# RoadlyInc/DSOPP

Measured on AMD Instinct MI355X. Metric: Gauss-Newton iters/sec (7-KF window, 2k active pts), higher is better.
Workload: dtype f64; 1 GPU; C1: 7-KF window, 2000 active points per GPU (2000 total, 2000 on rank 0), 640x480, full clique, production LM settings; frames=7, points_per_gpu=2000, total_points=2000, parallelism=single GPU, exchange=none, ranks=1

## Files before the change

### dsopp_amd/csrc/pba.hip

```cpp
#include <algorithm>
#include <chrono>
#include <cstdlib>
#include <map>
#include <memory>
#include <mutex>

#include "host_linalg.hpp"
#include "pba_solve_kernels.hpp"
#include "pba_solve_combined.hpp"
#include "pba_schur_two_stage.hpp"
#include "depth_map_kernels.hpp"
#include "point_status_kernels.hpp"
#include "depth_maps.hpp"
#include "activation_kernels.hpp"
#include "immature_set.hpp"
#include "semantic_observation_kernels.hpp"

namespace dsopp_hip {
namespace {

struct ResidualTable {
  DeviceBuffer<uint8_t> status, cand, fej_valid, snap_status;
  DeviceBuffer<double> energy;
  int n = 0, snap_n = 0;
};

struct HostFrame {
  int id = 0;
  int64_t timestamp = 0;
  const dsopp_hip_pyramid *pyramid = nullptr;
  unsigned pyramid_generation = 0;
  int level = 0;
  double intr[4] = {0, 0, 0, 0};
  double exposure = 1;
  bool fixed = false, is_marginalized = false, to_marginalize = false;
  int n = 0;
  int cap = 0;
  std::map<int, std::vector<uint8_t>> pending;
  std::vector<uint8_t> flags;
  DeviceBuffer<double> uv, idepth, idepth_step, idepth_fej, patch, inv_hdd, b_d, relative_baseline, ublk;
  DeviceBuffer<int32_t> n_inliers;
  DeviceBuffer<uint8_t> dflags, snap_flags;
  DeviceBuffer<double> snap_idepth;
  int snap_n = 0;
  std::map<int, std::unique_ptr<ResidualTable>> residuals;
  std::map<int, std::array<double, 36>> covariance;
  std::vector<int> to_internal, to_caller;
  std::vector<int> batch_end;
  DeviceBuffer<int> d_to_internal;
  bool permuted() const { return !to_internal.empty(); }
  DeviceBuffer<uint8_t> sem_hist;
  int internalOf(int caller) const { return to_internal.empty() ? caller : to_internal[static_cast<size_t>(caller)]; }
};

}
}

using namespace dsopp_hip;

struct dsopp_hip_window {
  StreamRef sr;
  dsopp_hip_options opt;
  std::vector<std::unique_ptr<HostFrame>> frames;
  WindowState hst;
  std::vector<double> Hm, bm;
  double energy_marginalized = 0;
  int marg_size = 0;
  DeviceBuffer<FrameDev> d_frames;
  DeviceBuffer<WindowState> d_state, d_state_snap;
  DeviceBuffer<PairConst> d_pc;
  DeviceBuffer<SweepBlock> d_sweep_table;
  DeviceBuffer<SweepBlock> d_fine_table;
  int n_fine_blocks = 0;
  const SweepBlock *fineTable() const { return d_fine_table.ptr ? d_fine_table.ptr : d_sweep_table.ptr; }
  DeviceBuffer<SchurBlock> d_schur_table;
  DeviceBuffer<int> d_pair_first, d_pair_count;
  DeviceBuffer<double> d_partials, d_reduce, d_Hpp, d_bpp, d_Hm, d_Hm_packed, d_bm, d_step, d_scalars, d_gather;
  bool marg_nonzero = false;
  DeviceBuffer<double> d_schur_partials, d_pair_out;
  bool deterministic = false;
  int twoStageMinChunks() const {
    static const int override_chunks = std::getenv("DSOPP_HIP_TWO_STAGE_MIN_CHUNKS") ? std::atoi(std::getenv("DSOPP_HIP_TWO_STAGE_MIN_CHUNKS")) : 0;
    if (override_chunks > 0) return override_chunks;
    return kTwoStageMinChunks;
  }
  bool twoStage() const { return deterministic || n_schur_blocks > twoStageMinChunks(); }
  DeviceMem<unsigned> d_bs_flag;
  unsigned bs_seq = 0, bs_ticket_base = 0;
  PinnedMem<int> h_bs_fault;
  DeviceMem<long long> dbg_stamps;
  DeviceMem<long long> dbg_sweep;
  bool dbg_sweep_lin = true;
  DeviceBuffer<LmControl> d_ctrl;
  const LmControl *fused_final_ctrl = nullptr;
  bool async_pending = false;
  bool begun_with_first_estimate = true;
  int lm_mode = 0;
  double *dHppRaw() const { return d_reduce.ptr; }
  double *dbppRaw() const { return d_reduce.ptr + static_cast<size_t>(K()) * K(); }
  double *dHsc() const { return dbppRaw() + K(); }
  double *dbsc() const { return dHsc() + static_cast<size_t>(K()) * K(); }
  void d_HscDownload(double *host, size_t n, size_t off, hipStream_t st) const {
    HIP_CHECK(hipMemcpyAsync(host, dHsc() + off, n * sizeof(double), hipMemcpyDeviceToHost, st));
  }
  void d_bscDownload(double *host, size_t n, size_t off, hipStream_t st) const {
    HIP_CHECK(hipMemcpyAsync(host, dbsc() + off, n * sizeof(double), hipMemcpyDeviceToHost, st));
  }
  size_t reduceCount() const { return 2 * (static_cast<size_t>(K()) * K() + K()); }
  size_t combCount() const { return static_cast<size_t>(combBlockCount(F())) * 64 + static_cast<size_t>(K()); }
  int comb_copies_active = 1;
  size_t combCopyFirst() const { return (combCount() + 4 * kScalarGroups + 8 + 1) & ~static_cast<size_t>(1); }
  size_t combCopyStride() const { return (combCount() + 1) & ~static_cast<size_t>(1); }
  int n_sweep_blocks = 0, n_schur_blocks = 0;
  bool topology_dirty = true;
  bool frames_dirty = false;
  std::vector<FrameDev> h_frames;
  bool state_dirty = true;
  bool host_stale = false;
  PinnedMem<LmControl> h_ctrl;
  PinnedMem<void> h_uncertainty;
  Event uncertainty_ready;
  bool restore_in_begin = false;
  DeviceBuffer<LmControl> d_results;
  PinnedMem<LmControl> h_results;
  LmControl *result_device = nullptr;
  DeviceBuffer<SelectState> d_select;
  DeviceBuffer<double> d_pair_dist;
  DeviceBuffer<double> d_export;
  PinnedMem<void> h_export;
  struct StageRing {
    PinnedMem<char> mem;
    size_t offset = 0;
  } stage;
  struct AppendOp {
    int kind;
    int n;
    int a;
    int first_block;
    unsigned long long src_off;
    void *dst;
    void *p[6];
  };
  std::vector<uint8_t> append_blob;
  std::vector<AppendOp> append_ops;
  DeviceBuffer<uint8_t> d_append;
  struct ExportEntry {
    int frame_id, n;
    size_t word_offset;
    std::vector<int> target_ids;
  };
  std::vector<ExportEntry> export_entries;
  DeviceBuffer<double> d_update;
  PinnedMem<void> h_update;
  bool export_valid = false;
  std::vector<std::unique_ptr<HostFrame>> frame_pool;
  std::vector<std::unique_ptr<ResidualTable>> table_pool;
  DeviceBuffer<uint8_t> d_sem_args;
  DeviceBuffer<double> dm_tmp;
  std::vector<dsopp_hip_depth_maps *> live_maps;
  struct ActivationScratch {
    DeviceBuffer<ActKeyframe> keyframes;
    DeviceBuffer<ActPair> pairs;
    DeviceBuffer<const void *> texels0;
    DeviceBuffer<double> px, py;
    DeviceBuffer<double> sx, sy;
    DeviceBuffer<int> state, cell_cursor, sid, accepted, nbr, nbr_count;
    DeviceBuffer<double> pack;
  } act;
  bool marg_dirty = true;
  bool pair_valid = false;
  bool begun = false;
  bool linearized = false;
  bool reduced_by_collective = false;
  double last_lambda = 0;
  std::vector<double> last_step;
  float last_solve_ms = 0;
  bool solve_events_pending = false;
  Event ev0, ev1;
  dsopp_hip_allreduce_fn allreduce = nullptr;
  void *allreduce_user = nullptr;
  int rank = 0, world = 1;
  bool profiling = false;
  struct TimedLaunch {
    int cls;
    Event a, b;
  };
  std::vector<TimedLaunch> timed;
  std::vector<Event> event_pool;
  double prof_ms[DSOPP_HIP_NUM_KERNEL_CLASSES] = {0};
  int64_t prof_count[DSOPP_HIP_NUM_KERNEL_CLASSES] = {0};
  WindowState snap_state;
  bool snap_valid = false;
  int snap_F = 0;

  int F() const { return static_cast<int>(frames.size()); }
  int K() const { return kBlk * F(); }
  bool fej() const { return opt.first_estimate_jacobians != 0; }
  int slotOf(int id) const {
    for (size_t i = 0; i < frames.size(); ++i)
      if (frames[i]->id == id) return static_cast<int>(i);
    return -1;
  }
  HostFrame &frameById(int id) {
    const int s = slotOf(id);
    if (s < 0) fail(DSOPP_HIP_ERR_NOT_FOUND, "frame %d is not in the window", id);
    return *frames[static_cast<size_t>(s)];
  }
};

namespace dsopp_hip {
namespace {

using W = dsopp_hip_window;

}
int nativeAllreduce(void *user, void *device_buffer, size_t count, void *stream);
namespace {

Event takeEvent(W &w) {
  Event e;
  if (!w.event_pool.empty()) {
    e = std::move(w.event_pool.back());
    w.event_pool.pop_back();
  } else {
    (void)e.get(hipEventDefault);
  }
  return e;
}

template <typename Body>
void timedLaunch(W &w, int cls, Body &&body) {
  if (!w.profiling) {
    body();
    return;
  }
  Event a = takeEvent(w), b = takeEvent(w);
  HIP_CHECK(hipEventRecord(a.h, w.sr.stream));
  body();
  HIP_CHECK(hipEventRecord(b.h, w.sr.stream));
  w.timed.push_back({cls, std::move(a), std::move(b)});
}

void collectTimings(W &w) {
  if (w.timed.empty()) return;
  w.sr.sync();
  for (auto &t : w.timed) {
    float ms = 0;
    HIP_CHECK(hipEventElapsedTime(&ms, t.a.h, t.b.h));
    w.prof_ms[t.cls] += ms;
    w.prof_count[t.cls] += 1;
    w.event_pool.push_back(std::move(t.a));
    w.event_pool.push_back(std::move(t.b));
  }
  w.timed.clear();
}

__global__ void gatherRowsKernel(const uint8_t *__restrict__ src, uint8_t *__restrict__ dst, const int *__restrict__ rows, int count, int row_bytes) {
  const long long e = static_cast<long long>(blockIdx.x) * blockDim.x + threadIdx.x;
  if (e >= static_cast<long long>(count) * row_bytes) return;
  const int k = static_cast<int>(e / row_bytes), b = static_cast<int>(e % row_bytes);
  dst[e] = src[static_cast<size_t>(rows[k]) * row_bytes + b];
}

void flushAppends(W &w, const char *why = "flush: in front of an entry point");

void splitBatchAt(W &w, HostFrame &f, int n) {
  if (!f.permuted() || n <= 0 || n >= f.n) return;
  int b0 = 0, b1 = f.n;
  for (int e : f.batch_end) {
    if (e == n) return;
    if (e < n) b0 = std::max(b0, e);
    if (e > n) b1 = std::min(b1, e);
  }
  flushAppends(w, "flush: splitBatchAt");
  const int count = b1 - b0;
  std::vector<int> new_to_old;
  new_to_old.reserve(static_cast<size_t>(count));
  for (int p = b0; p < b1; ++p)
    if (f.to_caller[static_cast<size_t>(p)] < n) new_to_old.push_back(p);
  for (int p = b0; p < b1; ++p)
    if (f.to_caller[static_cast<size_t>(p)] >= n) new_to_old.push_back(p);
  hipStream_t st = w.sr.stream;
  DeviceBuffer<int> d_rows;
  DeviceBuffer<uint8_t> tmp;
  d_rows.reserve(static_cast<size_t>(count), 0, st);
  d_rows.upload(new_to_old.data(), new_to_old.size(), 0, st);
  auto permute = [&](void *base, size_t row_bytes) {
    if (!base) return;
    const size_t bytes = static_cast<size_t>(count) * row_bytes;
    tmp.reserve(bytes, 0, st);
    gatherRowsKernel<<<static_cast<unsigned>((bytes + 255) / 256), 256, 0, st>>>(static_cast<const uint8_t *>(base), tmp.ptr, d_rows.ptr, count,
                                                                                 static_cast<int>(row_bytes));
    HIP_CHECK(hipGetLastError());
    HIP_CHECK(hipMemcpyAsync(static_cast<uint8_t *>(base) + static_cast<size_t>(b0) * row_bytes, tmp.ptr, bytes, hipMemcpyDeviceToDevice, st));
  };
  permute(f.uv.ptr, 2 * sizeof(double));
  permute(f.idepth.ptr, sizeof(double));
  permute(f.idepth_step.ptr, sizeof(double));
  permute(f.idepth_fej.ptr, sizeof(double));
  permute(f.patch.ptr, kPat * sizeof(double));
  permute(f.inv_hdd.ptr, sizeof(double));
  permute(f.b_d.ptr, sizeof(double));
  permute(f.relative_baseline.ptr, sizeof(double));
  permute(f.n_inliers.ptr, sizeof(int32_t));
  permute(f.dflags.ptr, 1);
  if (f.ublk.ptr)
    for (int pl = 0; pl < 2 * kMaxFrames; ++pl) permute(f.ublk.ptr + static_cast<size_t>(pl) * ublkPlane(f.cap), kUblk * sizeof(double));
  for (auto &kv : f.residuals) {
    ResidualTable &rt = *kv.second;
    if (rt.n < b1) continue;
    permute(rt.status.ptr, 1);
    permute(rt.cand.ptr, 1);
    permute(rt.fej_valid.ptr, 1);
    permute(rt.energy.ptr, sizeof(double));
  }
  f.snap_n = 0;
  for (auto &kv : f.residuals) kv.second->snap_n = 0;
  w.snap_valid = false;
  HIP_CHECK(hipStreamSynchronize(st));
  const std::vector<int> old_to_caller(f.to_caller.begin() + b0, f.to_caller.begin() + b1);
  for (int k = 0; k < count; ++k) {
    const int c = old_to_caller[static_cast<size_t>(new_to_old[static_cast<size_t>(k)] - b0)];
    f.to_caller[static_cast<size_t>(b0 + k)] = c;
    f.to_internal[static_cast<size_t>(c)] = b0 + k;
  }
  f.batch_end.push_back(n);
  f.d_to_internal.upload(f.to_internal.data(), f.to_internal.size(), 0, st);
  HIP_CHECK(hipStreamSynchronize(st));
  w.linearized = false;
  w.export_valid = false;
}

constexpr int kFirstLandmarkCapacity = 2048;

void ensureLandmarkCapacity(W &w, HostFrame &f, int n) {
  if (n <= f.cap) return;
  flushAppends(w, "flush: landmark arrays grow");
  int cap = f.cap ? f.cap : kFirstLandmarkCapacity;
  while (cap < n) cap *= 2;
  hipStream_t st = w.sr.stream;
  const size_t keep = static_cast<size_t>(f.n);
  f.uv.reserve(2 * static_cast<size_t>(cap), 2 * keep, st);
  f.idepth.reserve(cap, keep, st);
  f.idepth_step.reserve(cap, keep, st);
  f.idepth_fej.reserve(cap, keep, st);
  f.patch.reserve(static_cast<size_t>(kPat) * cap, kPat * keep, st);
  f.inv_hdd.reserve(cap, keep, st);
  f.b_d.reserve(cap, keep, st);
  f.relative_baseline.reserve(cap, keep, st);
  f.n_inliers.reserve(cap, keep, st);
  f.dflags.reserve(cap, keep, st);
  f.ublk.reserve(2 * static_cast<size_t>(kMaxFrames) * ublkPlane(cap), 0, st);
  for (auto &kv : f.residuals) {
    ResidualTable &rt = *kv.second;
    const size_t k = static_cast<size_t>(rt.n);
    rt.status.reserve(cap, k, st);
    rt.cand.reserve(cap, k, st);
    rt.fej_valid.reserve(cap, k, st);
    rt.energy.reserve(cap, k, st);
  }
  f.cap = cap;
  w.topology_dirty = true;
}

void reserveGeometric(PinnedMem<void> &buf, size_t need) {
  if (need <= buf.bytes) return;
  size_t cap = std::max<size_t>(buf.bytes, size_t(1) << 16);
  while (cap < need) cap *= 2;
  buf.reserve(cap);
}

void *stageAcquire(W &w, size_t bytes) {
  bytes = (bytes + 63) & ~static_cast<size_t>(63);
  if (bytes > w.stage.mem.bytes) {
    if (w.stage.mem) {
      w.sr.sync();
      w.stage.mem.reset();
    }
    w.stage.mem.reserve(std::max<size_t>(bytes * 2, size_t(1) << 21));
    w.stage.offset = 0;
  }
  if (w.stage.offset + bytes > w.stage.mem.bytes) {
    w.sr.sync();
    w.stage.offset = 0;
  }
  void *p = w.stage.mem.get() + w.stage.offset;
  w.stage.offset += bytes;
  return p;
}
constexpr int kAppendBlockElems = 2048;

__global__ void __launch_bounds__(256) applyAppendsKernel(const uint8_t *__restrict__ blob, const W::AppendOp *__restrict__ ops, int n_ops) {
  __shared__ int s_op;
  if (threadIdx.x == 0) {
    int lo = 0;
    for (int i = 1; i < n_ops; ++i)
      if (ops[i].first_block <= static_cast<int>(blockIdx.x)) lo = i;
    s_op = lo;
  }
  __syncthreads();
  const W::AppendOp op = ops[s_op];
  const int chunk = static_cast<int>(blockIdx.x) - op.first_block;
  const uint8_t *src = blob + op.src_off;
  const int e0 = chunk * kAppendBlockElems, e1 = e0 + kAppendBlockElems < op.n ? e0 + kAppendBlockElems : op.n;
  if (op.kind == 0) {
    if (op.a == 8) {
      for (int i = e0 + static_cast<int>(threadIdx.x); i < e1; i += 256) static_cast<unsigned long long *>(op.dst)[i] = reinterpret_cast<const unsigned long long *>(src)[i];
    } else if (op.a == 4) {
      for (int i = e0 + static_cast<int>(threadIdx.x); i < e1; i += 256) static_cast<unsigned *>(op.dst)[i] = reinterpret_cast<const unsigned *>(src)[i];
    } else {
      for (int i = e0 + static_cast<int>(threadIdx.x); i < e1; i += 256) static_cast<uint8_t *>(op.dst)[i] = src[i];
    }
    return;
  }
  if (op.kind == 1) {
// ... 2 lines not shown
      const uint8_t h = src[i];
      if (i < op.a) {
        dflags[i] = static_cast<uint8_t>((dflags[i] & (kFlagOutlier | kFlagIllConditioned)) | (h & (kFlagMarginalized | kFlagToMarginalize)));
      } else {
        dflags[i] = h;
        if (op.p[0]) {
          static_cast<double *>(op.p[0])[i] = 0;
          static_cast<double *>(op.p[1])[i] = 0;
          static_cast<double *>(op.p[2])[i] = 0;
          static_cast<double *>(op.p[3])[i] = 0;
          static_cast<double *>(op.p[4])[i] = 0;
          static_cast<int32_t *>(op.p[5])[i] = 0;
        }
      }
    }
    return;
  }
  if (op.kind == 4) {
    const SweepBlock tmpl = *reinterpret_cast<const SweepBlock *>(src);
    const int step = op.a, first = static_cast<int>(reinterpret_cast<intptr_t>(op.p[0])), n_all = static_cast<int>(reinterpret_cast<intptr_t>(op.p[1]));
    SweepBlock *out = static_cast<SweepBlock *>(op.dst);
    for (int k = e0 + static_cast<int>(threadIdx.x); k < e1; k += 256) {
      SweepBlock sb = tmpl;
      sb.offset = k * step * kItemsPerBlock;
      sb.n_groups = n_all ? (step < n_all - k * step ? step : n_all - k * step) : 1;
      sb.partial_row = first + k;
      out[k] = sb;
    }
    return;
  }
  if (op.kind == 3) {
    uint8_t *dflags = static_cast<uint8_t *>(op.dst);
    for (int i = e0 + static_cast<int>(threadIdx.x); i < e1; i += 256) dflags[i] &= static_cast<uint8_t>(~op.a);
    return;
  }
  for (int i = e0 + static_cast<int>(threadIdx.x); i < e1; i += 256) {
    const uint8_t st = src[i];
    const size_t j = static_cast<size_t>(op.a) + static_cast<size_t>(i);
    static_cast<uint8_t *>(op.dst)[j] = st;
    static_cast<uint8_t *>(op.p[0])[j] = st;
    static_cast<uint8_t *>(op.p[1])[j] = 0;
    static_cast<double *>(op.p[2])[j] = 0;
  }
}

void flushAppends(W &w, const char *why) {
  if (w.append_ops.empty()) return;
  HostTimes ht_(why);
  const int n_ops = static_cast<int>(w.append_ops.size());
  int blocks = 0;
  for (W::AppendOp &op : w.append_ops) {
    op.first_block = blocks;
    blocks += (op.n + kAppendBlockElems - 1) / kAppendBlockElems;
  }
  const size_t data_bytes = (w.append_blob.size() + 15) & ~static_cast<size_t>(15), table_bytes = static_cast<size_t>(n_ops) * sizeof(W::AppendOp);
  hipStream_t st = w.sr.stream;
  w.d_append.reserve(data_bytes + table_bytes, 0, st);
  uint8_t *p = static_cast<uint8_t *>(stageAcquire(w, data_bytes + table_bytes));
  std::memcpy(p, w.append_blob.data(), w.append_blob.size());
  std::memcpy(p + data_bytes, w.append_ops.data(), table_bytes);
  HIP_CHECK(hipMemcpyAsync(w.d_append.ptr, p, data_bytes + table_bytes, hipMemcpyHostToDevice, st));
  applyAppendsKernel<<<static_cast<unsigned>(blocks), 256, 0, st>>>(w.d_append.ptr, reinterpret_cast<const W::AppendOp *>(w.d_append.ptr + data_bytes), n_ops);
  HIP_CHECK(hipGetLastError());
  w.append_blob.clear();
  w.append_ops.clear();
}

size_t queueAppendData(W &w, const void *host, size_t bytes, const void *dst_a, const void *dst_b = nullptr) {
  for (const W::AppendOp &op : w.append_ops)
    if (op.dst == dst_a || (dst_b && op.dst == dst_b)) {
      flushAppends(w, "flush: a queued operation writes the same array");
      break;
    }
  const size_t off = (w.append_blob.size() + 7) & ~static_cast<size_t>(7);
  w.append_blob.resize(off + bytes);
  if (bytes) std::memcpy(w.append_blob.data() + off, host, bytes);
  return off;
}

void uploadStagedBytes(W &w, void *dst, const void *host, size_t bytes) {
  if (!bytes) return;
  W::AppendOp op{};
  op.kind = 0;
  const bool words = (bytes & 7) == 0 && (reinterpret_cast<uintptr_t>(dst) & 7) == 0;
  const bool half = (bytes & 3) == 0 && (reinterpret_cast<uintptr_t>(dst) & 3) == 0;
  op.a = words ? 8 : (half ? 4 : 1);
  op.n = static_cast<int>(bytes / static_cast<size_t>(op.a));
  op.src_off = queueAppendData(w, host, bytes, dst);
  op.dst = dst;
  w.append_ops.push_back(op);
}

template <typename T>
void uploadStaged(W &w, DeviceBuffer<T> &dst, const T *host, size_t count, size_t offset) {
  if (!count) return;
  static_assert(sizeof(T) == 8 || sizeof(T) == 4 || sizeof(T) == 1, "element size of a queued copy");
  W::AppendOp op{};
  op.kind = 0;
  op.n = static_cast<int>(count);
  op.a = static_cast<int>(sizeof(T));
  op.src_off = queueAppendData(w, host, count * sizeof(T), dst.ptr + offset);
  op.dst = dst.ptr + offset;
  w.append_ops.push_back(op);
}


void syncTopology(W &w) {
  HostTimes ht_("syncTopology");
  if (!w.topology_dirty) {
    if (w.frames_dirty && w.h_frames.size() == static_cast<size_t>(kMaxFrames) && w.d_frames.ptr) {
      for (int r = 0; r < w.F(); ++r) {
        w.h_frames[static_cast<size_t>(r)].is_marginalized = w.frames[static_cast<size_t>(r)]->is_marginalized;
        w.h_frames[static_cast<size_t>(r)].to_marginalize = w.frames[static_cast<size_t>(r)]->to_marginalize;
      }
      uploadStagedBytes(w, w.d_frames.ptr, w.h_frames.data(), static_cast<size_t>(kMaxFrames) * sizeof(FrameDev));
    }
    w.frames_dirty = false;
    return;
  }
  hipStream_t st = w.sr.stream;
  const int F = w.F();
  static thread_local std::vector<FrameDev> fd;
  static thread_local std::vector<SchurBlock> schur;
  static thread_local std::vector<SweepBlock> pair_tmpl;
  static thread_local std::vector<int> pair_items;
  fd.assign(static_cast<size_t>(kMaxFrames), FrameDev{});
  std::memset(fd.data(), 0, fd.size() * sizeof(FrameDev));
  schur.clear();
  pair_tmpl.resize(kMaxFrames * kMaxFrames);
  pair_items.assign(kMaxFrames * kMaxFrames, 0);
  size_t total_items = 0;
  for (int r = 0; r < F; ++r)
    for (const auto &kv : w.frames[static_cast<size_t>(r)]->residuals) total_items += static_cast<size_t>(kv.second->n);
  const int groups = total_items >= 300000 ? 6 : (total_items >= 30000 ? 4 : 1);
  std::vector<int> pair_first(kMaxFrames * kMaxFrames, -1), pair_count(kMaxFrames * kMaxFrames, 0);
  for (int r = 0; r < F; ++r) {
    HostFrame &f = *w.frames[static_cast<size_t>(r)];
    FrameDev &d = fd[static_cast<size_t>(r)];
    const LevelView lv = f.pyramid->view(f.level);
    d.texels = hbm(lv.texels);
    d.iplane = hbm(f.pyramid->intensityPlane(f.level, st));
    f.pyramid_generation = f.pyramid->generation;
    d.itiles = f.pyramid->itilesX(f.level);
    d.width = lv.width;
    d.height = lv.height;
    d.fx = f.intr[0];
    d.fy = f.intr[1];
    d.cx = f.intr[2];
    d.cy = f.intr[3];
    d.exposure = f.exposure;
    d.fixed = f.fixed;
    d.is_marginalized = f.is_marginalized;
    d.to_marginalize = f.to_marginalize;
    d.n = f.n;
    d.cap = f.cap;
    d.uv = hbm(f.uv.ptr);
    d.idepth = hbm(f.idepth.ptr);
    d.idepth_step = hbm(f.idepth_step.ptr);
    d.idepth_fej = hbm(f.idepth_fej.ptr);
    d.patch = hbm(f.patch.ptr);
    d.inv_hdd = hbm(f.inv_hdd.ptr);
    d.b_d = hbm(f.b_d.ptr);
    d.relative_baseline = hbm(f.relative_baseline.ptr);
    d.n_inliers = hbm(f.n_inliers.ptr);
    d.flags = hbm(f.dflags.ptr);
    d.ublk = hbm(f.ublk.ptr);
    d.snap_idepth = hbm(f.snap_idepth.ptr);
    d.snap_flags = hbm(f.snap_flags.ptr);
    d.first_conn = -1;
    for (int t = 0; t < F; ++t) {
      if (t == r) continue;
      auto it = f.residuals.find(w.frames[static_cast<size_t>(t)]->id);
      if (it == f.residuals.end() || it->second->n == 0) continue;
      ResidualTable &rt = *it->second;
      d.status[t] = hbm(rt.status.ptr);
      d.cand[t] = hbm(rt.cand.ptr);
      d.fej_valid[t] = hbm(rt.fej_valid.ptr);
      d.energy[t] = hbm(rt.energy.ptr);
      d.n_res[t] = rt.n;
      d.snap_status[t] = hbm(rt.snap_status.ptr);
      if (d.first_conn < 0) d.first_conn = t;
      SweepBlock sb;
      std::memset(&sb, 0, sizeof(sb));
      sb.r = r;
      sb.t = t;
      sb.n_res = rt.n;
      sb.cap = f.cap;
      sb.owns_landmark_sums = d.first_conn == t ? 1 : 0;
      sb.width_r = lv.width;
      sb.height_r = lv.height;
      sb.uv = d.uv;
      sb.idepth = d.idepth;
      sb.patch = d.patch;
      sb.idepth_fej = d.idepth_fej;
      sb.b_d = d.b_d;
      sb.inv_hdd = d.inv_hdd;
      sb.idepth_step = d.idepth_step;
      sb.ublk = d.ublk;
      sb.energy = hbm(rt.energy.ptr);
      sb.flags = d.flags;
      sb.status = hbm(rt.status.ptr);
      sb.fej_valid = hbm(rt.fej_valid.ptr);
      sb.cand = hbm(rt.cand.ptr);
      sb.n_groups = 1;
      pair_tmpl[static_cast<size_t>(r * kMaxFrames + t)] = sb;
      pair_items[static_cast<size_t>(r * kMaxFrames + t)] = (rt.n + kItemsPerBlock - 1) / kItemsPerBlock;
    }
    for (int off = 0; off < f.n; off += kSchurLandmarks) {
      SchurBlock sb;
      std::memset(&sb, 0, sizeof(sb));
      sb.r = r;
      sb.offset = off;
      sb.n = d.n;
      sb.cap = d.cap;
      sb.fixed = d.fixed;
      sb.idepth = d.idepth;
      sb.idepth_step = d.idepth_step;
      sb.inv_hdd = d.inv_hdd;
      sb.b_d = d.b_d;
      sb.ublk = d.ublk;
      sb.flags = d.flags;
      for (int t = 0; t < F; ++t) {
        if (d.status[t] == nullptr) continue;
        sb.conn_mask |= 1u << t;
        sb.status[t] = d.status[t];
        sb.cand[t] = d.cand[t];
        sb.n_res[t] = d.n_res[t];
      }
      schur.push_back(sb);
    }
  }
  const int step = groups > 1 ? groups : 1;
  struct PairRange {
    size_t pi;
    int first_sweep, n_sweep, first_fine, n_fine;
  };
  static thread_local std::vector<PairRange> ranges;
  ranges.clear();
  int total_sweep = 0, total_fine = 0;
  for (int t = 0; t < F; ++t)
    for (int r = 0; r < F; ++r) {
      const size_t pi = static_cast<size_t>(r * kMaxFrames + t);
      const int n_all = pair_items[pi];
      if (n_all == 0) continue;
      SweepBlock &tm = pair_tmpl[pi];
      const FrameDev &dr = fd[static_cast<size_t>(r)], &dt = fd[static_cast<size_t>(t)];
      tm.width_t = dt.width;
      tm.height_t = dt.height;
      tm.texels_t = dt.texels;
      tm.iplane_t = dt.iplane;
      tm.itiles_t = dt.itiles;
      for (int k = 0; k < F; ++k)
        if (dr.status[k] != nullptr) tm.conn_mask |= 1u << k;
      const int n_sweep = (n_all + step - 1) / step;
      pair_first[pi] = total_sweep;
      pair_count[pi] = n_sweep;
      ranges.push_back({pi, total_sweep, n_sweep, total_fine, groups > 1 ? n_all : 0});
      total_sweep += n_sweep;
      total_fine += groups > 1 ? n_all : 0;
    }
  w.d_frames.reserve(kMaxFrames, 0, st);
  uploadStagedBytes(w, w.d_frames.ptr, fd.data(), (kMaxFrames) * sizeof(*w.d_frames.ptr));
  w.h_frames = fd;
  w.frames_dirty = false;
  auto queuePairEntries = [&](SweepBlock *table, const SweepBlock &tmpl, int first, int count, int entry_step, int n_all_for_groups) {
    W::AppendOp op{};
    op.kind = 4;
    op.n = count;
    op.a = entry_step;
    op.src_off = queueAppendData(w, &tmpl, sizeof(SweepBlock), table + first);
    op.dst = table + first;
    op.p[0] = reinterpret_cast<void *>(static_cast<intptr_t>(first));
    op.p[1] = reinterpret_cast<void *>(static_cast<intptr_t>(n_all_for_groups));
    w.append_ops.push_back(op);
  };
  const size_t n_sweep_entries = static_cast<size_t>(total_sweep);
  w.n_sweep_blocks = static_cast<int>(n_sweep_entries);
  w.n_schur_blocks = static_cast<int>(schur.size());
  if (n_sweep_entries > w.d_sweep_table.capacity || (groups > 1 && static_cast<size_t>(total_fine) > w.d_fine_table.capacity))
    flushAppends(w, "flush: sweep tables grow");
  w.d_sweep_table.reserve(std::max<size_t>(1, n_sweep_entries), 0, st);
  for (const PairRange &pr : ranges)
    queuePairEntries(w.d_sweep_table.ptr, pair_tmpl[pr.pi], pr.first_sweep, pr.n_sweep, step, groups > 1 ? pair_items[pr.pi] : 0);
  if (groups > 1) {
    w.d_fine_table.reserve(std::max<size_t>(1, static_cast<size_t>(total_fine)), 0, st);
    for (const PairRange &pr : ranges) queuePairEntries(w.d_fine_table.ptr, pair_tmpl[pr.pi], pr.first_fine, pr.n_fine, 1, 0);
    w.n_fine_blocks = total_fine;
  } else {
    w.d_fine_table.release();
    w.n_fine_blocks = static_cast<int>(n_sweep_entries);
  }
  w.d_schur_table.reserve(std::max<size_t>(1, schur.size()), 0, st);
  uploadStagedBytes(w, w.d_schur_table.ptr, schur.data(), (schur.size()) * sizeof(*w.d_schur_table.ptr));
  w.d_pair_first.reserve(kMaxFrames * kMaxFrames, 0, st);
  uploadStagedBytes(w, w.d_pair_first.ptr, pair_first.data(), (pair_first.size()) * sizeof(*w.d_pair_first.ptr));
  w.d_pair_count.reserve(kMaxFrames * kMaxFrames, 0, st);
  uploadStagedBytes(w, w.d_pair_count.ptr, pair_count.data(), (pair_count.size()) * sizeof(*w.d_pair_count.ptr));
  w.d_partials.reserve(std::max<size_t>(1, n_sweep_entries) * kPartial, 0, st);
  w.d_pc.reserve(kMaxFrames * kMaxFrames, 0, st);
  w.d_ctrl.reserve(2, 0, st);
  const size_t KK = static_cast<size_t>(kBlk * kMaxFrames);
  w.d_Hpp.reserve(2 * KK * KK, 0, st);
  w.d_bpp.reserve(KK, 0, st);
  w.d_reduce.reserve(2 * (KK * KK + KK) + 8 + 4 * kScalarGroups + 16 + static_cast<size_t>(kMaxCombCopies - 1) * (static_cast<size_t>(combBlockCount(kMaxFrames)) * 64 + KK + 2), 0, st);
  w.d_Hm.reserve(KK * KK, 0, st);
  w.d_bm.reserve(KK, 0, st);
  w.d_step.reserve(KK, 0, st);
  w.d_scalars.reserve(16 + 4 * kScalarGroups, 0, st);
  w.topology_dirty = false;
  w.pair_valid = false;
}

void uploadState(W &w) {
  if (!w.state_dirty) return;
  w.d_state.reserve(1, 0, w.sr.stream);
  uploadStagedBytes(w, w.d_state.ptr, &w.hst, sizeof(WindowState));
  w.state_dirty = false;
  w.pair_valid = false;
}

void downloadState(W &w) {
  if (w.state_dirty || !w.d_state.ptr || !w.host_stale) return;
  w.host_stale = false;
  w.d_state.download(&w.hst, 1, 0, w.sr.stream);
  w.sr.sync();
}

void uploadMarginal(W &w) {
  if (!w.marg_dirty) return;
  const int K = w.K();
  if (w.marg_size != K) fail(DSOPP_HIP_ERR_STATE, "marginal prior has size %d, window %d", w.marg_size, K);
  w.marg_nonzero = w.energy_marginalized != 0;
  for (double v : w.Hm) w.marg_nonzero = w.marg_nonzero || v != 0;
  for (double v : w.bm) w.marg_nonzero = w.marg_nonzero || v != 0;
  uploadStagedBytes(w, w.d_Hm.ptr, w.Hm.data(), static_cast<size_t>(K) * K * sizeof(double));
  uploadStagedBytes(w, w.d_bm.ptr, w.bm.data(), static_cast<size_t>(K) * sizeof(double));
  const int F = w.F();
  std::vector<double> packed(static_cast<size_t>(combBlockCount(F)) * 64);
  for (int bi = 0; bi < F; ++bi)
    for (int bj = 0; bj <= bi; ++bj)
      for (int i = 0; i < kBlk; ++i)
        for (int j = 0; j < kBlk; ++j)
          packed[static_cast<size_t>(combBlockIndex(bi, bj)) * 64 + static_cast<size_t>(i * kBlk + j)] =
              w.Hm[static_cast<size_t>(kBlk * bi + i) * K + static_cast<size_t>(kBlk * bj + j)];
  w.d_Hm_packed.reserve(static_cast<size_t>(combBlockCount(kMaxFrames)) * 64, 0, w.sr.stream);
  uploadStagedBytes(w, w.d_Hm_packed.ptr, packed.data(), packed.size() * sizeof(double));
  w.marg_dirty = false;
}

void checkPyramidGenerations(W &w) {
  for (const auto &fp : w.frames)
    if (fp->pyramid && fp->pyramid->generation != fp->pyramid_generation) w.topology_dirty = true;
}

void prepare(W &w) {
  w.sr.use();
  checkPyramidGenerations(w);
  downloadState(w);
  syncTopology(w);
  uploadState(w);
  uploadMarginal(w);
  flushAppends(w, "flush: prepare()");
}

void prepareDevice(W &w) {
  w.sr.use();
  flushAppends(w);
  checkPyramidGenerations(w);
  if (w.state_dirty || w.topology_dirty || w.frames_dirty || w.marg_dirty || !w.d_state.ptr) prepare(w);
}

void ensurePairConstants(W &w) {
  if (w.pair_valid) return;
  const int F = w.F();
  timedLaunch(w, DSOPP_HIP_KERNEL_PAIR_SETUP, [&] {
    pairSetupKernel<<<1, kMaxFrames * kMaxFrames, 0, w.sr.stream>>>(w.d_frames.ptr, w.d_state.ptr, w.d_pc.ptr, F, w.fej() ? 1 : 0, nullptr);
  });
  HIP_CHECK(hipGetLastError());
  w.pair_valid = true;
}

template <typename S>
void launchFej(W &w) {
  if (!w.n_sweep_blocks) return;
  timedLaunch(w, DSOPP_HIP_KERNEL_FEJ,
              [&] {
                const int per_wave = 64 / kItemsPerBlock;
                fejKernel<S><<<(w.n_fine_blocks + per_wave - 1) / per_wave, 64, 0, w.sr.stream>>>(w.d_frames.ptr, w.d_pc.ptr, w.fineTable(),
                                                                                                  w.n_fine_blocks);
              });
  HIP_CHECK(hipGetLastError());
}

void firstEstimate(W &w) {
  ensurePairConstants(w);
  if (w.opt.dtype == DSOPP_HIP_F64)
    launchFej<double>(w);
  else
    launchFej<float>(w);
}

struct SweepExtras {
  int ublk_read = 0, ublk_write = 0;
  bool gate_on_pending = false;
  const int *run_flag = nullptr;
  bool fused_lin_backsub = false;
  bool combined = false;
  bool external_backsub = false;
  bool write_fej = false;
};

template <typename S>
void launchSweepTyped(W &w, bool lin, bool huber, bool for_marg, const LmControl *ctrl, bool backsub, double lambda, const SweepExtras &ex) {
  if (!w.n_sweep_blocks) {
    if (lin) HIP_CHECK(hipMemsetAsync(w.d_reduce.ptr, 0, w.reduceCount() * sizeof(double), w.sr.stream));
    return;
  }
  SweepParams prm;
  prm.sigma_huber = w.opt.sigma_huber_loss;
  prm.for_marginalized = for_marg ? 1 : 0;
  prm.use_fej_flag = w.fej() ? 1 : 0;
  prm.ctrl = ctrl;
  prm.clear_buf = lin ? w.d_reduce.ptr : nullptr;
  prm.clear_count = static_cast<int>(ex.combined ? w.combCount() + 4 : w.reduceCount());
  if (ex.combined && w.comb_copies_active > 1)
    prm.clear_count = static_cast<int>(w.combCopyFirst() + (w.comb_copies_active - 1) * w.combCopyStride());
  prm.step = w.d_step.ptr;
  prm.lambda = lambda;
  prm.F = w.F();
  prm.ublk_read = ex.ublk_read;
  prm.ublk_write = ex.ublk_write;
  prm.gate_on_pending = ex.gate_on_pending ? 1 : 0;
  prm.run_flag = ex.run_flag;
  prm.external_backsub = ex.external_backsub ? 1 : 0;
  prm.dbg = (w.dbg_sweep && lin == w.dbg_sweep_lin) ? w.dbg_sweep.get() : nullptr;
  dim3 grid(static_cast<unsigned>(w.n_sweep_blocks)), block(kSweepThreads);
  hipStream_t st = w.sr.stream;
  const FrameDev *fr = w.d_frames.ptr;
  const PairConst *pc = w.d_pc.ptr;
  const SweepBlock *tb = w.d_sweep_table.ptr;
  double *pa = w.d_partials.ptr;
  const bool opening = lin && huber && ex.write_fej && w.fej();
  if (opening) prm.external_backsub = 1;
  timedLaunch(w, lin ? DSOPP_HIP_KERNEL_SWEEP_LINEARIZE : DSOPP_HIP_KERNEL_SWEEP_ENERGY, [&] {
    if (opening) {
      sweepKernel<S, true, true, true, false, true><<<grid, block, 0, st>>>(fr, pc, tb, pa, prm.ctrl, prm.run_flag, prm);
    } else if (lin && ex.fused_lin_backsub) {
      if (w.fej())
        sweepKernel<S, true, true, true, true><<<grid, block, 0, st>>>(fr, pc, tb, pa, prm.ctrl, prm.run_flag, prm);
      else
        sweepKernel<S, true, false, true, true><<<grid, block, 0, st>>>(fr, pc, tb, pa, prm.ctrl, prm.run_flag, prm);
    } else if (!lin && backsub) {
      if (w.fej())
        sweepKernel<S, false, true, true, true><<<grid, block, 0, st>>>(fr, pc, tb, pa, prm.ctrl, prm.run_flag, prm);
      else
        sweepKernel<S, false, false, true, true><<<grid, block, 0, st>>>(fr, pc, tb, pa, prm.ctrl, prm.run_flag, prm);
    } else if (!lin) {
      if (w.fej())
        sweepKernel<S, false, true, true><<<grid, block, 0, st>>>(fr, pc, tb, pa, prm.ctrl, prm.run_flag, prm);
      else
        sweepKernel<S, false, false, true><<<grid, block, 0, st>>>(fr, pc, tb, pa, prm.ctrl, prm.run_flag, prm);
    } else if (w.fej()) {
      if (huber)
        sweepKernel<S, true, true, true><<<grid, block, 0, st>>>(fr, pc, tb, pa, prm.ctrl, prm.run_flag, prm);
      else
        sweepKernel<S, true, true, false><<<grid, block, 0, st>>>(fr, pc, tb, pa, prm.ctrl, prm.run_flag, prm);
    } else {
      if (huber)
        sweepKernel<S, true, false, true><<<grid, block, 0, st>>>(fr, pc, tb, pa, prm.ctrl, prm.run_flag, prm);
      else
        sweepKernel<S, true, false, false><<<grid, block, 0, st>>>(fr, pc, tb, pa, prm.ctrl, prm.run_flag, prm);
    }
  });
  HIP_CHECK(hipGetLastError());
}

void launchSweep(W &w, bool lin, bool huber, bool for_marg, const LmControl *ctrl = nullptr, bool backsub = false, double lambda = 0,
                 const SweepExtras &ex = SweepExtras()) {
  if (!ctrl && !ex.run_flag) ensurePairConstants(w);
  backsub = backsub && w.opt.optimize_idepths;
  if (w.opt.dtype == DSOPP_HIP_F64)
    launchSweepTyped<double>(w, lin, huber, for_marg, ctrl, backsub, lambda, ex);
  else
    launchSweepTyped<float>(w, lin, huber, for_marg, ctrl, backsub, lambda, ex);
}

void allreduceIfNeeded(W &w, double *dev, size_t count) {
  if (!w.allreduce) return;
  const int rc = w.allreduce(w.allreduce_user, dev, count, w.sr.stream);
  if (rc != 0) fail(DSOPP_HIP_ERR_HIP, "allreduce callback failed with %d", rc);
}

size_t schurSmemBytes(int K) {
  const int Kp = (K + 15) & ~15;
  return (static_cast<size_t>(kSchurLandmarks) * schurRowStride(Kp) + 2 * kSchurLandmarks + 40 * static_cast<size_t>(kMaxFrames)) * sizeof(double);
}

struct FusedReduce {
  int ublk_parity;
  LmControl *ctrl_out;
  LmParams prm;
  bool combined = false;
  double comb_lambda = 0;
  const double *scalars = nullptr;
  LmControl *ctrl_host = nullptr;
};

enum class ReduceMode { kFused, kAccumulateOnly, kDecideOnly };
constexpr size_t kDecideSmemBytes = size_t((6 * (kSchurThreads + 2) + 6 * 72) * 8);

void launchTwoStage(W &w, const LmControl *ctrl, int ublk_parity, double lambda, bool dense, double *group_sums);
void launchReduceSchur(W &w, bool for_marg, const LmControl *ctrl, const FusedReduce *fused = nullptr, ReduceMode mode = ReduceMode::kFused) {
  const int K = w.K(), F = w.F();
  hipStream_t st = w.sr.stream;
  if (!fused && !for_marg && !ctrl && w.deterministic) {
    launchTwoStage(w, nullptr, 0, 0.0, true, nullptr);
    allreduceIfNeeded(w, w.d_reduce.ptr, w.reduceCount());
    return;
  }
  ensureDynamicLds(reinterpret_cast<const void *>(reduceSchurKernel), w.sr.device, 96 * 1024);
  ReduceSchurArgs a;
  a.frames = w.d_frames.ptr;
  a.pc = w.d_pc.ptr;
  a.schur_table = w.d_schur_table.ptr;
  a.partials = w.d_partials.ptr;
  a.pair_first_block = w.d_pair_first.ptr;
  a.pair_num_blocks = w.d_pair_count.ptr;
  a.Hpp = w.dHppRaw();
  a.bpp = w.dbppRaw();
  a.Hsc = w.dHsc();
  a.bsc = w.dbsc();
  a.ctrl = ctrl;
  a.F = F;
  a.n_schur_blocks = w.opt.optimize_idepths ? w.n_schur_blocks : 0;
  a.for_marginalized = for_marg ? 1 : 0;
  a.ublk_parity = fused ? fused->ublk_parity : 0;
  a.ctrl_out = (fused && mode != ReduceMode::kAccumulateOnly) ? fused->ctrl_out : nullptr;
  a.st = w.d_state.ptr;
  const bool combined = fused && fused->combined;
  const size_t reduce_count = combined ? w.combCount() : w.reduceCount();
  a.comb = combined ? w.d_reduce.ptr : nullptr;
  a.comb_lambda = fused ? fused->comb_lambda : 0.0;
  if (combined && mode == ReduceMode::kAccumulateOnly && w.comb_copies_active > 1) {
    a.comb_copies = w.comb_copies_active;
    a.comb_copy_first = static_cast<int>(w.combCopyFirst());
    a.comb_copy_stride = static_cast<int>(w.combCopyStride());
  }
  a.scalars = mode == ReduceMode::kDecideOnly ? w.d_reduce.ptr + reduce_count : w.d_scalars.ptr;
  a.n_sweep_blocks = w.n_sweep_blocks;
  a.total_blocks = a.n_schur_blocks + F * F;
  a.scalars_out = mode == ReduceMode::kAccumulateOnly ? w.d_reduce.ptr + reduce_count : nullptr;
  const bool grouped_tail = mode == ReduceMode::kAccumulateOnly && w.allreduce != nullptr;
  a.scalars_out_groups = grouped_tail ? kScalarGroups : 0;
  static_assert(4 * kScalarGroups <= kSchurThreads, "one workgroup writes the grouped tail");
  if (fused) a.prm = fused->prm;
  if (fused && fused->scalars) a.scalars = fused->scalars;
  a.ctrl_host = fused ? fused->ctrl_host : nullptr;
  a.dbg = w.dbg_stamps ? w.dbg_stamps.get() + 24 : nullptr;
  const size_t decide_smem = kDecideSmemBytes;
  if (mode == ReduceMode::kDecideOnly) {
    timedLaunch(w, DSOPP_HIP_KERNEL_ACCEPT,
                [&] { decideApplyKernel<<<std::max(1, a.n_schur_blocks), kSchurThreads, decide_smem, st>>>(a); });
    HIP_CHECK(hipGetLastError());
    return;
  }
  timedLaunch(w, DSOPP_HIP_KERNEL_SCHUR, [&] {
    reduceSchurKernel<<<a.n_schur_blocks + F * F + (a.scalars_out ? 1 : 0), kSchurThreads, std::max(schurSmemBytes(K), decide_smem), st>>>(
        a.ctrl, a.schur_table, a.pc, a.partials, a.pair_first_block, a.pair_num_blocks, a.n_schur_blocks, a.F, a);
  });
  HIP_CHECK(hipGetLastError());
  allreduceIfNeeded(w, w.d_reduce.ptr, reduce_count + (mode == ReduceMode::kAccumulateOnly ? (grouped_tail ? 4 * kScalarGroups : 4) : 0));
  (void)K;
}

SolveArgs makeSolveArgs(W &w) {
  SolveArgs a;
  a.frames = w.d_frames.ptr;
  a.st = w.d_state.ptr;
  a.pc = w.d_pc.ptr;
  a.Hpp_raw = w.dHppRaw();
  a.bpp_raw = w.dbppRaw();
  a.Hpp_out = w.d_Hpp.ptr;
  a.Hsc_copy = w.d_Hpp.ptr + static_cast<size_t>(w.K()) * w.K();
  a.bpp_out = w.d_bpp.ptr;
  a.Hsc = w.dHsc();
  a.bsc = w.dbsc();
  a.use_marginal = w.marg_nonzero ? 1 : 0;
  a.Hm = w.d_Hm.ptr;
  a.bm = w.d_bm.ptr;
  a.step = w.d_step.ptr;
  a.lambda = 0;
  a.affine_reg[0] = w.opt.affine_brightness_regularizer[0];
  a.affine_reg[1] = w.opt.affine_brightness_regularizer[1];
  a.fixed_reg = w.opt.fixed_state_regularizer;
  a.energy_marginalized = w.energy_marginalized;
  a.F = w.F();
  a.fej = w.fej() ? 1 : 0;
  a.do_solve = 1;
  a.store_system = 0;
  a.add_priors = 1;
  return a;
}

size_t solveSmemBytes(int K) {
  const size_t N = static_cast<size_t>(K) + 1;
  return (N * (N + 1) + 4 * static_cast<size_t>(K) + 32 + 38 * static_cast<size_t>(kMaxFrames)) * sizeof(double);
}

void launchAssemble(W &w, double lambda, bool do_solve, bool add_priors, bool store_system) {
  ensureDynamicLds(reinterpret_cast<const void *>(assembleSolveKernel), w.sr.device, 150 * 1024);
  SolveArgs a = makeSolveArgs(w);
  a.lambda = lambda;
  a.do_solve = do_solve ? 1 : 0;
  a.add_priors = add_priors ? 1 : 0;
  a.store_system = store_system ? 1 : 0;
  timedLaunch(w, do_solve ? DSOPP_HIP_KERNEL_ASSEMBLE_SOLVE : DSOPP_HIP_KERNEL_ASSEMBLE,
              [&] { assembleSolveKernel<<<1, kSolveThreads, solveSmemBytes(w.K()), w.sr.stream>>>(a); });
  if (do_solve && !w.fej()) {
    pairSetupKernel<<<1, kMaxFrames * kMaxFrames, 0, w.sr.stream>>>(w.d_frames.ptr, w.d_state.ptr, w.d_pc.ptr, w.F(), 0, nullptr);
  }
  HIP_CHECK(hipGetLastError());
}

void launchTwoStage(W &w, const LmControl *ctrl, int ublk_parity, double lambda, bool dense = false, double *group_sums = nullptr) {
  const int F = w.F();
  hipStream_t st = w.sr.stream;
  using TwoStageKernel = void (*)(TwoStageArgs);
  static const TwoStageKernel kernels[6] = {nullptr, schurTwoStageKernel<2>, schurTwoStageKernel<2>, schurTwoStageKernel<3>, schurTwoStageKernel<4>,
                                            schurTwoStageKernel<5>};
  const int tpw = twoStageTilesPerWave(F);
  if (tpw < 1 || tpw > kMaxTilesPerWave) fail(DSOPP_HIP_ERR_CAPACITY, "window of %d frames exceeds the Schur kernel's tile budget", F);
  const TwoStageKernel two_stage_kernel = kernels[tpw];
  ensureDynamicLds(reinterpret_cast<const void *>(two_stage_kernel), w.sr.device, 96 * 1024);
  const int n_chunks = w.opt.optimize_idepths ? w.n_schur_blocks : 0;
  const int n_wgs = std::max(1, std::min(512, n_chunks));
  w.d_schur_partials.reserve(std::max<size_t>(1, static_cast<size_t>(n_wgs)) * static_cast<size_t>(twoStagePartialCount(F)), 0, st);
  w.d_pair_out.reserve(static_cast<size_t>(kMaxFrames) * kMaxFrames * kPairOut, 0, st);
  TwoStageArgs a;
  a.frames = w.d_frames.ptr;
  a.pc = w.d_pc.ptr;
  a.schur_table = w.d_schur_table.ptr;
  a.partials = w.d_partials.ptr;
  a.dbg = w.dbg_stamps ? w.dbg_stamps.get() + 32 : nullptr;
  a.pair_first_block = w.d_pair_first.ptr;
  a.pair_num_blocks = w.d_pair_count.ptr;
  a.ctrl = ctrl;
  a.schur_partials = w.d_schur_partials.ptr;
  a.pair_out = w.d_pair_out.ptr;
  a.F = F;
  a.n_chunks = n_chunks;
  a.n_schur_wgs = n_wgs;
  a.ublk_parity = ublk_parity;
  a.group_sums = group_sums;
  a.n_sweep_blocks = w.n_sweep_blocks;
  CombineArgs c;
  c.pc = w.d_pc.ptr;
  c.schur_partials = w.d_schur_partials.ptr;
  c.pair_out = w.d_pair_out.ptr;
  c.ctrl = ctrl;
  c.lambda = lambda;
  c.comb = w.d_reduce.ptr;
  c.dense = dense ? w.d_reduce.ptr : nullptr;
  c.F = F;
  c.n_schur_wgs = n_wgs;
  const size_t pair_smem = (48 + 64 + kPairBlk + 8 * 48) * sizeof(double);
  timedLaunch(w, DSOPP_HIP_KERNEL_SCHUR, [&] {
    two_stage_kernel<<<n_wgs + F * F + (group_sums ? kScalarGroups : 0), kSchurThreads, std::max(twoStageSmemBytes(F), pair_smem), st>>>(a);
    combineSystemKernel<<<static_cast<unsigned>((twoStagePartialCount(F) + kCombineEntries - 1) / kCombineEntries), kCombineEntries * kCombineSlices, 0, st>>>(c);
  });
  HIP_CHECK(hipGetLastError());
}

int solveResidentWorkgroups(W &w, bool wide) {
  static std::map<std::pair<int, size_t>, int> cache;
  static std::mutex mu;
  const size_t smem = solveSmemBytes(w.K());
  std::lock_guard<std::mutex> lock(mu);
  const auto key = std::make_pair(w.sr.device * 2 + (wide ? 1 : 0), smem);
  auto it = cache.find(key);
  if (it != cache.end()) return it->second;
  int per_cu = 0, cus = 0;
  if (wide)
    HIP_CHECK(hipOccupancyMaxActiveBlocksPerMultiprocessor(&per_cu, solveCombinedKernel<512>, 512, smem));
  else
    HIP_CHECK(hipOccupancyMaxActiveBlocksPerMultiprocessor(&per_cu, solveCombinedKernel<256>, 256, smem));
  HIP_CHECK(hipDeviceGetAttribute(&cus, hipDeviceAttributeMultiprocessorCount, w.sr.device));
  const int n = std::max(2, per_cu * cus);
  cache[key] = n;
  return n;
}

void launchSolveCombined(W &w, double lambda, LmControl *ctrl, const LmControl *decide_from = nullptr, const LmParams *decide_prm = nullptr,
                         bool decide_from_groups = false, bool backsub = false, int ublk_parity = 0) {
  ensureDynamicLds(reinterpret_cast<const void *>(solveCombinedKernel<256>), w.sr.device, 150 * 1024);
  ensureDynamicLds(reinterpret_cast<const void *>(solveCombinedKernel<256, kMaxCombCopies>), w.sr.device, 150 * 1024);
  ensureDynamicLds(reinterpret_cast<const void *>(solveCombinedKernel<512>), w.sr.device, 150 * 1024);
  SolveCombArgs a;
  if (decide_from) {
    a.dec_in = decide_from;
    a.dec_scalars = w.d_reduce.ptr + w.combCount();
    a.dec_table = w.d_schur_table.ptr;
    a.dec_chunks = w.n_schur_blocks;
    const bool wide = w.F() > 8;
    a.dec_blocks = std::min(wide ? (w.n_schur_blocks + 1) / 2 : w.n_schur_blocks, solveResidentWorkgroups(w, wide) - 1);
    a.dec_groups = decide_from_groups ? kScalarGroups : 0;
    a.dec_prm = *decide_prm;
    if (backsub && a.dec_blocks > 0) {
      if (!w.d_bs_flag) {
        constexpr size_t kHand = static_cast<size_t>(kBlk) * kMaxFrames;
        w.d_bs_flag.alloc(16 + 2 * kHand * sizeof(double));
        std::vector<double> arm(2 * kHand, kHandOverSentinel());
        HIP_CHECK(hipMemsetAsync(w.d_bs_flag.get(), 0, 16, w.sr.stream));
        HIP_CHECK(hipMemcpyAsync(reinterpret_cast<char *>(w.d_bs_flag.get()) + 16, arm.data(), arm.size() * sizeof(double), hipMemcpyHostToDevice, w.sr.stream));
        HIP_CHECK(hipStreamSynchronize(w.sr.stream));
        w.h_bs_fault.reserve(sizeof(int));
        *w.h_bs_fault.get() = 0;
      }
      {
        constexpr size_t kHand = static_cast<size_t>(kBlk) * kMaxFrames;
        double *hand = reinterpret_cast<double *>(reinterpret_cast<char *>(w.d_bs_flag.get()) + 16);
        const unsigned n = w.bs_seq;
        a.bs_ticket = w.d_bs_flag.get();
        a.bs_hand = hand + (n & 1u) * kHand;
        a.bs_hand_next = hand + ((n + 1) & 1u) * kHand;
      }
      a.bs_parity = ublk_parity;
      a.bs_ticket_base = w.bs_ticket_base;
      a.bs_fault = w.h_bs_fault.get();
    }
  }
  a.frames = w.d_frames.ptr;
  a.st = w.d_state.ptr;
  a.pc = w.d_pc.ptr;
  a.comb = w.d_reduce.ptr;
  if (w.comb_copies_active > 1) {
    a.comb_copies = w.comb_copies_active;
    a.comb_copy_first = static_cast<int>(w.combCopyFirst());
    a.comb_copy_stride = static_cast<int>(w.combCopyStride());
  }
  a.Hm = w.d_Hm.ptr;
  a.HmPacked = w.d_Hm_packed.ptr;
  a.bm = w.d_bm.ptr;
  a.step = w.d_step.ptr;
  a.ctrl = ctrl;
  a.lambda = lambda;
  a.affine_reg[0] = w.opt.affine_brightness_regularizer[0];
  a.affine_reg[1] = w.opt.affine_brightness_regularizer[1];
  a.fixed_reg = w.opt.fixed_state_regularizer;
  a.energy_marginalized = w.energy_marginalized;
  a.F = w.F();
  a.fej = w.fej() ? 1 : 0;
  a.use_marginal = w.marg_nonzero ? 1 : 0;
  a.dbg_stamps = w.dbg_stamps.get();
  timedLaunch(w, DSOPP_HIP_KERNEL_ASSEMBLE_SOLVE,
              [&] {
                if (w.F() > 8)
                  solveCombinedKernel<512><<<1 + a.dec_blocks, 512, solveSmemBytes(w.K()), w.sr.stream>>>(
                      a.bs_ticket, a.bs_hand_next, a.dec_in, a.dec_scalars, a.comb, a.frames, a.st, a.F, a);
                else if (a.comb_copies > 1)
                  solveCombinedKernel<256, kMaxCombCopies><<<1 + a.dec_blocks, 256, solveSmemBytes(w.K()), w.sr.stream>>>(
                      a.bs_ticket, a.bs_hand_next, a.dec_in, a.dec_scalars, a.comb, a.frames, a.st, a.F, a);
                else
                  solveCombinedKernel<256><<<1 + a.dec_blocks, 256, solveSmemBytes(w.K()), w.sr.stream>>>(
                      a.bs_ticket, a.bs_hand_next, a.dec_in, a.dec_scalars, a.comb, a.frames, a.st, a.F, a);
              });
  HIP_CHECK(hipGetLastError());
  if (a.bs_ticket) {
    w.bs_seq++;
    w.bs_ticket_base += static_cast<unsigned>(1 + a.dec_blocks);
  }
  if (!w.fej()) {
    pairSetupKernel<<<1, kMaxFrames * kMaxFrames, 0, w.sr.stream>>>(w.d_frames.ptr, w.d_state.ptr, w.d_pc.ptr, w.F(), 0, nullptr);
    HIP_CHECK(hipGetLastError());
  }
}

void checkSolveLaunchFault(W &w) {
  if (!w.h_bs_fault || !*w.h_bs_fault.get()) return;
  *w.h_bs_fault.get() = 0;
  constexpr size_t kHand = static_cast<size_t>(kBlk) * kMaxFrames;
  std::vector<double> arm(2 * kHand, kHandOverSentinel());
  HIP_CHECK(hipMemsetAsync(w.d_bs_flag.get(), 0, 16, w.sr.stream));
  HIP_CHECK(hipMemcpyAsync(reinterpret_cast<char *>(w.d_bs_flag.get()) + 16, arm.data(), arm.size() * sizeof(double), hipMemcpyHostToDevice, w.sr.stream));
  HIP_CHECK(hipStreamSynchronize(w.sr.stream));
  w.bs_seq = 0;
  w.bs_ticket_base = 0;
  fail(DSOPP_HIP_ERR_HIP, "a solve launch's landmark workgroups waited 2 s for the pose step (device shared with a kernel that never yields?): "
                          "the inverse depths of that iteration were not updated, the solve is void");
}

void launchBacksub(W &w, double lambda, const LmControl *ctrl, int ublk_parity = 0, bool gate_on_pending = false) {
  if (!w.opt.optimize_idepths || !w.n_schur_blocks) return;
  timedLaunch(w, DSOPP_HIP_KERNEL_BACKSUB, [&] {
    backsubKernel<<<w.n_schur_blocks, kSchurLandmarks, 0, w.sr.stream>>>(w.d_frames.ptr, w.d_schur_table.ptr, w.d_step.ptr, lambda, w.F(), ctrl,
                                                                         ublk_parity, gate_on_pending ? 1 : 0);
  });
  HIP_CHECK(hipGetLastError());
}


double priorEnergy(const W &w, bool with_step) {
  const int F = w.F(), K = w.K();
  std::vector<double> state(static_cast<size_t>(K));
  for (int f = 0; f < F; ++f)
    for (int a = 0; a < kBlk; ++a) state[static_cast<size_t>(kBlk * f + a)] = w.hst.eps[f][a] + (with_step ? w.hst.step[f][a] : 0.0);
  double e = w.energy_marginalized;
  double quad = 0, lin = 0;
  for (int i = 0; i < K; ++i) {
    lin += w.bm[static_cast<size_t>(i)] * state[static_cast<size_t>(i)];
    double s = 0;
    for (int j = 0; j < K; ++j) s += w.Hm[static_cast<size_t>(i) * K + j] * state[static_cast<size_t>(j)];
    quad += state[static_cast<size_t>(i)] * s;
  }
  e += lin + quad / 2;
  for (int f = 0; f < F; ++f) {
    double t = 0;
    for (int a = 0; a < 2; ++a) {
      const double ab = w.hst.ab0[f][a] + state[static_cast<size_t>(kBlk * f + 6 + a)];
      t += ab * w.opt.affine_brightness_regularizer[a] * ab;
    }
    e += t / 2;
  }
  return e;
}

void stageBegin(W &w) {
  if (w.F() == 0) fail(DSOPP_HIP_ERR_STATE, "window is empty");
  prepare(w);
  if (w.fej()) firstEstimate(w);
  w.begun_with_first_estimate = true;
  w.begun = true;
  w.linearized = false;
}

void fusedBegin(W &w) {
  if (w.F() == 0) fail(DSOPP_HIP_ERR_STATE, "window is empty");
  if (!(w.fej() && w.opt.max_iterations > 0)) {
    stageBegin(w);
    return;
  }
  prepare(w);
  w.begun_with_first_estimate = false;
  w.begun = true;
  w.linearized = false;
}

std::pair<double, int> stageEnergy(W &w) {
  if (!w.begun) fail(DSOPP_HIP_ERR_STATE, "call begin first");
  launchSweep(w, false, true, false);
  timedLaunch(w, DSOPP_HIP_KERNEL_ENERGY_REDUCE,
              [&] { energyReduceKernel<<<1, 256, 0, w.sr.stream>>>(w.d_partials.ptr, w.n_sweep_blocks, w.d_scalars.ptr); });
  HIP_CHECK(hipGetLastError());
  allreduceIfNeeded(w, w.d_scalars.ptr, 2);
  double out[2];
  w.d_scalars.download(out, 2, 0, w.sr.stream);
  w.sr.sync();
  return {out[0] + priorEnergy(w, true), static_cast<int>(out[1] + 0.5)};
}

void stageLinearize(W &w, bool huber = true, bool for_marg = false, bool add_priors = true) {
  if (!w.begun) fail(DSOPP_HIP_ERR_STATE, "call begin first");
  launchSweep(w, true, huber, for_marg);
  launchReduceSchur(w, for_marg, nullptr);
  launchAssemble(w, 0.0, false, add_priors, true);
  w.linearized = true;
}

void stageStep(W &w, double lambda) {
  if (!w.linearized) fail(DSOPP_HIP_ERR_STATE, "call linearize first");
  launchAssemble(w, lambda, true, true, false);
  w.pair_valid = true;
  launchBacksub(w, lambda, nullptr);
  const int K = w.K();
  w.last_step.resize(static_cast<size_t>(K));
  w.d_step.download(w.last_step.data(), static_cast<size_t>(K), 0, w.sr.stream);
  w.sr.sync();
  for (int f = 0; f < w.F(); ++f)
    for (int a = 0; a < kBlk; ++a) w.hst.step[f][a] = -w.last_step[static_cast<size_t>(kBlk * f + a)];
  w.last_lambda = lambda;
}

std::pair<double, double> stageAccept(W &w, bool accept) {
  HIP_CHECK(hipMemsetAsync(w.d_scalars.ptr + 4, 0, 4 * sizeof(double), w.sr.stream));
  timedLaunch(w, DSOPP_HIP_KERNEL_ACCEPT, [&] {
    if (w.n_schur_blocks) {
      acceptLandmarksKernel<<<w.n_schur_blocks, kSchurThreads, 0, w.sr.stream>>>(w.d_frames.ptr, w.d_schur_table.ptr, w.F(), accept ? 1 : 0,
                                                                                  w.d_scalars.ptr + 4);
    }
    acceptFramesKernel<<<1, 128, 0, w.sr.stream>>>(w.d_state.ptr, w.F(), accept ? 1 : 0, w.d_scalars.ptr + 6);
  });
  HIP_CHECK(hipGetLastError());
  if (accept) allreduceIfNeeded(w, w.d_scalars.ptr + 4, 2);
  double n4[4];
  w.d_scalars.download(n4, 4, 4, w.sr.stream);
  w.sr.sync();
  const double norms[2] = {n4[0] + n4[2], n4[1] + n4[3]};
  for (int f = 0; f < w.F(); ++f)
    for (int a = 0; a < kBlk; ++a) {
      if (accept) w.hst.eps[f][a] += w.hst.step[f][a];
      w.hst.step[f][a] = 0;
    }
  if (!accept) w.pair_valid = false;
  return {norms[0], norms[1]};
}

void restoreHostSide(W &w) {
  if (!w.snap_valid || w.snap_F != w.F()) fail(DSOPP_HIP_ERR_STATE, "no snapshot matching the current window");
  w.sr.use();
  flushAppends(w);
  for (auto &fp : w.frames) {
    if (fp->snap_n != fp->n) fail(DSOPP_HIP_ERR_STATE, "frame %d changed since the snapshot", fp->id);
    for (auto &kv : fp->residuals)
      if (kv.second->snap_n != kv.second->n) fail(DSOPP_HIP_ERR_STATE, "connection of frame %d changed since the snapshot", fp->id);
  }
  syncTopology(w);
  flushAppends(w);
  w.hst = w.snap_state;
  w.state_dirty = false;
  w.host_stale = false;
  w.pair_valid = false;
  w.begun = false;
}

void launchRestore(W &w) {
  restoreKernel<<<w.n_schur_blocks + 1, kSchurLandmarks, 0, w.sr.stream>>>(w.d_frames.ptr, w.d_schur_table.ptr, w.F(), w.d_state.ptr, w.d_state_snap.ptr,
                                                                        w.n_schur_blocks);
  HIP_CHECK(hipGetLastError());
}

void lmSolveFusedEnqueue(W &w) {
  hipStream_t st = w.sr.stream;
  LmParams prm;
  prm.function_tolerance = w.opt.function_tolerance;
  prm.parameter_tolerance = w.opt.parameter_tolerance;
  prm.decrease_on_accept = 1.0;
  prm.increase_on_reject = 1.0;
  prm.lambda0 = 1.0 / w.opt.initial_trust_region_radius;
  prm.max_iterations = w.opt.max_iterations;
  prm.min_iterations = 3;
  prm.force_accept = w.opt.force_accept;
  prm.use_reduced_scalars = w.allreduce ? 1 : 0;
  LmControl *ctrl = w.d_ctrl.ptr;
  const bool sweep_takes_fej = w.fej() && w.opt.max_iterations > 0 && !w.begun_with_first_estimate;
  const bool begin_sets_pairs = !w.pair_valid;
  {
    LmInitArgs ia;
    ia.pair_frames = begin_sets_pairs ? w.d_frames.ptr : nullptr;
    ia.pair_pc = w.d_pc.ptr;
    ia.pair_fej = w.fej() ? 1 : 0;
    w.pair_valid = true;
    ia.sa = makeSolveArgs(w);
    ia.schur_table = w.d_schur_table.ptr;
    ia.n_schur_blocks = w.n_schur_blocks;
    ia.ctrl = ctrl;
    ia.prm = prm;
    int begin_blocks = 1;
    if (w.restore_in_begin) {
      w.restore_in_begin = false;
      if (begin_sets_pairs) {
        ia.restore_state = w.d_state.ptr;
        ia.sa.st = w.d_state_snap.ptr;
        begin_blocks += w.n_schur_blocks + 1;
      } else {
        launchRestore(w);
      }
    }
    lmBeginKernel<<<begin_blocks, kSolveThreads, (static_cast<size_t>(w.K()) + 16) * sizeof(double), st>>>(ia);
  }
  HIP_CHECK(hipGetLastError());
  const int rounds = (w.opt.force_accept ? w.opt.max_iterations : 2 * w.opt.max_iterations) + 1;
  bool result_written_by_kernel = false;
  const bool k3_backsub = w.opt.optimize_idepths && w.n_schur_blocks > 0;
  static const int comb_copies_min_chunks = std::getenv("DSOPP_HIP_COMB_COPIES_MIN_CHUNKS") ? std::atoi(std::getenv("DSOPP_HIP_COMB_COPIES_MIN_CHUNKS")) : 80;
  w.comb_copies_active = (!w.twoStage() && !w.allreduce && w.F() <= 7 && w.n_schur_blocks >= comb_copies_min_chunks) ? kMaxCombCopies : 1;
  struct CopiesReset {
    W &w;
    ~CopiesReset() { w.comb_copies_active = 1; }
  } copies_reset{w};
  for (int r = 0; r < rounds; ++r) {
    LmControl *cin = ctrl + (r & 1), *cout = ctrl + ((r + 1) & 1);
    SweepExtras ex;
    ex.ublk_read = (r + 1) & 1;
    ex.ublk_write = r & 1;
    ex.gate_on_pending = true;
    ex.fused_lin_backsub = true;
    ex.combined = true;
    ex.write_fej = r == 0 && sweep_takes_fej;
    const bool large = w.n_schur_blocks > w.twoStageMinChunks();
    if (k3_backsub) {
      ex.fused_lin_backsub = false;
      ex.external_backsub = true;
      launchSweep(w, r + 1 < rounds, true, false, cin, false, 0.0, ex);
    } else if (large && r + 1 == rounds) {
      launchBacksub(w, 0.0, cin, ex.ublk_read, true);
      ex.fused_lin_backsub = false;
      ex.external_backsub = true;
      launchSweep(w, false, true, false, cin, false, 0.0, ex);
    } else if (large) {
      if (r > 0) launchBacksub(w, 0.0, cin, ex.ublk_read, true);
      ex.fused_lin_backsub = false;
      ex.external_backsub = true;
      launchSweep(w, true, true, false, cin, false, 0.0, ex);
    } else {
      launchSweep(w, r + 1 < rounds, true, false, cin, true, 0.0, ex);
    }
    FusedReduce fr;
    fr.ublk_parity = r & 1;
    fr.ctrl_out = cout;
    fr.prm = prm;
    fr.combined = true;
    bool decide_from_groups = false;
    if (w.twoStage() && r + 1 < rounds) {
      double *groups = w.d_reduce.ptr + w.combCount();
      launchTwoStage(w, cin, fr.ublk_parity, 0.0, false, groups);
      allreduceIfNeeded(w, w.d_reduce.ptr, w.combCount() + 4 * kScalarGroups);
      decide_from_groups = true;
    } else if (w.allreduce && r + 1 == rounds) {
      if (large) {
        sweepScalarGroupsKernel<<<kScalarGroups, 256, 0, st>>>(w.d_partials.ptr, w.n_sweep_blocks, w.d_scalars.ptr + 16, cin);
        sweepScalarGroupsFinalKernel<<<1, 64, 0, st>>>(w.d_scalars.ptr + 16, w.d_reduce.ptr + w.combCount());
      } else {
        sweepScalarsKernel<<<1, 256, 0, st>>>(w.d_partials.ptr, w.n_sweep_blocks, w.d_reduce.ptr + w.combCount(), cin);
      }
      HIP_CHECK(hipGetLastError());
      allreduceIfNeeded(w, w.d_reduce.ptr + w.combCount(), 4);
      launchReduceSchur(w, false, cin, &fr, ReduceMode::kDecideOnly);
    } else if (r + 1 == rounds) {
      w.h_ctrl.reserve(sizeof(LmControl));
      fr.ctrl_host = w.result_device ? w.result_device : w.h_ctrl.get();
      result_written_by_kernel = true;
      if (large) {
        sweepScalarGroupsKernel<<<kScalarGroups, 256, 0, st>>>(w.d_partials.ptr, w.n_sweep_blocks, w.d_scalars.ptr + 16, cin);
        HIP_CHECK(hipGetLastError());
        fr.prm.use_reduced_scalars = 2;
        fr.scalars = w.d_scalars.ptr + 16;
      }
      launchReduceSchur(w, false, cin, &fr, ReduceMode::kDecideOnly);
    } else {
      launchReduceSchur(w, false, cin, &fr, ReduceMode::kAccumulateOnly);
      decide_from_groups = w.allreduce != nullptr;
    }
    if (r + 1 < rounds) launchSolveCombined(w, 0.0, cout, cin, &fr.prm, decide_from_groups, k3_backsub, fr.ublk_parity);
  }
  LmControl *cfin = ctrl + (rounds & 1);
  HIP_CHECK(hipGetLastError());
  w.pair_valid = false;
  w.h_ctrl.reserve(sizeof(LmControl));
  if (!result_written_by_kernel) {
    if (w.result_device)
      HIP_CHECK(hipMemcpyAsync(w.result_device, cfin, sizeof(LmControl), hipMemcpyDeviceToDevice, st));
    else
      HIP_CHECK(hipMemcpyAsync(w.h_ctrl.get(), cfin, sizeof(LmControl), hipMemcpyDeviceToHost, st));
  }
  w.host_stale = true;
  w.fused_final_ctrl = cfin;
}

void lmSolveFusedFinish(W &w, double &energy_out, int &iterations, int &n_valid_out) {
  hipStream_t st = w.sr.stream;
  const LmControl *cfin = w.fused_final_ctrl;
  w.sr.sync();
  checkSolveLaunchFault(w);
  if (w.h_ctrl.get()->need_final_setup) {
    ensurePairConstants(w);
    launchSweep(w, false, true, false);
    HIP_CHECK(hipGetLastError());
    w.sr.sync();
  }
  (void)st;
  (void)cfin;
  energy_out = w.h_ctrl.get()->energy;
  iterations = w.h_ctrl.get()->iteration;
  n_valid_out = w.h_ctrl.get()->n_valid;
}

void lmSolveFused(W &w, double &energy_out, int &iterations, int &n_valid_out) {
  lmSolveFusedEnqueue(w);
  lmSolveFusedFinish(w, energy_out, iterations, n_valid_out);
}

}
}

namespace dsopp_hip {
namespace {

Rigid poseOf(const W &w, int f) {
  Rigid T0;
  for (int i = 0; i < 9; ++i) T0.R[i] = w.hst.T0_R[f][i];
  for (int i = 0; i < 3; ++i) T0.t[i] = w.hst.T0_t[f][i];
  return rigidMul(T0, rigidExp(w.hst.eps[f]));
}

void relinearize(W &w) {
  prepareDevice(w);
  relinearizeKernel<<<1, kMaxFrames * kMaxFrames, 0, w.sr.stream>>>(w.d_frames.ptr, w.d_state.ptr, w.d_pc.ptr, w.F(), w.fej() ? 1 : 0, w.F() - 1);
  HIP_CHECK(hipGetLastError());
  w.host_stale = true;
  w.pair_valid = true;
}

void updatePointStatusesDevice(W &w) {
  prepareDevice(w);
  hipStream_t st = w.sr.stream;
  const int F = w.F();
  if (!w.d_select.ptr) {
    w.d_select.reserve(1, 0, st);
    selectInitKernel<<<1, 1024, 0, st>>>(w.d_select.ptr);
  }
  w.d_pair_dist.reserve(static_cast<size_t>(kMaxFrames) * kMaxFrames, 0, st);
  const double half_sigma_sq = w.opt.sigma_huber_loss * w.opt.sigma_huber_loss / 2;
  if (w.n_sweep_blocks) {
    const int per_group = kSelectThreads / kItemsPerBlock;
    const int grid = (w.n_fine_blocks + per_group - 1) / per_group;
    for (int pass = kSelectPasses - 1; pass >= 0; --pass)
      selectHistKernel<<<grid, kSelectThreads, 0, st>>>(w.d_frames.ptr, w.fineTable(), w.n_fine_blocks, w.d_select.ptr, pass);
  }
  pairDistanceKernel<<<1, 256, 0, st>>>(w.d_state.ptr, F, w.d_pair_dist.ptr, w.n_sweep_blocks ? w.d_select.ptr : nullptr, half_sigma_sq);
  if (w.n_schur_blocks)
    applyPointStatusesKernel<<<w.n_schur_blocks, kSchurLandmarks, 0, st>>>(w.d_frames.ptr, w.d_schur_table.ptr, F, w.d_select.ptr, w.d_pair_dist.ptr);
  HIP_CHECK(hipGetLastError());
}

void updatePointStatuses(W &w) {
  if (!(w.allreduce && w.world > 1)) {
    updatePointStatusesDevice(w);
    return;
  }
  prepare(w);
  downloadState(w);
  const int F = w.F();
  hipStream_t st = w.sr.stream;
  struct Conn {
    int r, t;
    std::vector<uint8_t> status, cand;
    std::vector<double> energy;
  };
  std::vector<Conn> conns;
  std::vector<std::vector<uint8_t>> flags(static_cast<size_t>(F));
  std::vector<std::vector<double>> idepth(static_cast<size_t>(F)), baseline(static_cast<size_t>(F));
  for (int r = 0; r < F; ++r) {
    HostFrame &f = *w.frames[static_cast<size_t>(r)];
    flags[static_cast<size_t>(r)].resize(static_cast<size_t>(f.n));
    idepth[static_cast<size_t>(r)].resize(static_cast<size_t>(f.n));
    baseline[static_cast<size_t>(r)].resize(static_cast<size_t>(f.n));
    f.dflags.download(flags[static_cast<size_t>(r)].data(), static_cast<size_t>(f.n), 0, st);
    f.idepth.download(idepth[static_cast<size_t>(r)].data(), static_cast<size_t>(f.n), 0, st);
    f.relative_baseline.download(baseline[static_cast<size_t>(r)].data(), static_cast<size_t>(f.n), 0, st);
    for (int t = 0; t < F; ++t) {
      if (t == r) continue;
      HostFrame &g = *w.frames[static_cast<size_t>(t)];
      if (g.is_marginalized) continue;
      auto it = f.residuals.find(g.id);
      if (it == f.residuals.end() || it->second->n == 0) continue;
      Conn c;
      c.r = r;
      c.t = t;
      c.status.resize(static_cast<size_t>(it->second->n));
      c.cand.resize(static_cast<size_t>(it->second->n));
      c.energy.resize(static_cast<size_t>(it->second->n));
      it->second->status.download(c.status.data(), c.status.size(), 0, st);
      it->second->cand.download(c.cand.data(), c.cand.size(), 0, st);
      it->second->energy.download(c.energy.data(), c.energy.size(), 0, st);
      conns.push_back(std::move(c));
    }
  }
  w.sr.sync();
  std::vector<double> energies;
  for (const Conn &c : conns)
    for (size_t i = 0; i < c.status.size(); ++i) {
      if (flags[static_cast<size_t>(c.r)][i] & kFlagMarginalized) continue;
      if (c.status[i] == DSOPP_HIP_STATUS_OK) energies.push_back(c.energy[i]);
    }
  if (w.allreduce && w.world > 1) {
    std::vector<double> counts(static_cast<size_t>(w.world), 0.0);
    counts[static_cast<size_t>(w.rank)] = static_cast<double>(energies.size());
    w.d_gather.reserve(static_cast<size_t>(w.world), 0, st);
    w.d_gather.upload(counts.data(), counts.size(), 0, st);
    allreduceIfNeeded(w, w.d_gather.ptr, counts.size());
    w.d_gather.download(counts.data(), counts.size(), 0, st);
    w.sr.sync();
    size_t total = 0, offset = 0;
    for (int r = 0; r < w.world; ++r) {
      if (r < w.rank) offset += static_cast<size_t>(counts[static_cast<size_t>(r)] + 0.5);
      total += static_cast<size_t>(counts[static_cast<size_t>(r)] + 0.5);
    }
    std::vector<double> all(total, 0.0);
    std::copy(energies.begin(), energies.end(), all.begin() + static_cast<long>(offset));
    if (total) {
      w.d_gather.reserve(total, 0, st);
      w.d_gather.upload(all.data(), total, 0, st);
      allreduceIfNeeded(w, w.d_gather.ptr, total);
      w.d_gather.download(all.data(), total, 0, st);
      w.sr.sync();
    }
    energies.swap(all);
  }
  double threshold = 0;
  if (!energies.empty()) {
    const size_t q = static_cast<size_t>(static_cast<double>(energies.size()) * 0.75);
    std::nth_element(energies.begin(), energies.begin() + static_cast<long>(q), energies.end());
    threshold = energies[q] + w.opt.sigma_huber_loss * w.opt.sigma_huber_loss / 2;
  }
  std::vector<std::vector<int32_t>> inliers(static_cast<size_t>(F));
  std::vector<std::vector<int>> valid(static_cast<size_t>(F));
  for (int r = 0; r < F; ++r) {
    inliers[static_cast<size_t>(r)].assign(static_cast<size_t>(w.frames[static_cast<size_t>(r)]->n), 0);
    valid[static_cast<size_t>(r)].assign(static_cast<size_t>(w.frames[static_cast<size_t>(r)]->n), 0);
  }
  for (Conn &c : conns) {
    const Rigid Tr = poseOf(w, c.r), Tt = poseOf(w, c.t);
    const double dx = Tr.t[0] - Tt.t[0], dy = Tr.t[1] - Tt.t[1], dz = Tr.t[2] - Tt.t[2];
    const double distance = std::sqrt(dx * dx + dy * dy + dz * dz);
    for (size_t i = 0; i < c.status.size(); ++i) {
      if (flags[static_cast<size_t>(c.r)][i] & kFlagMarginalized) continue;
      if (c.energy[i] > threshold) {
        c.status[i] = DSOPP_HIP_STATUS_OUTLIER;
        c.cand[i] = DSOPP_HIP_STATUS_OUTLIER;
        c.energy[i] = 0;
      }
      if (c.status[i] == DSOPP_HIP_STATUS_OK) {
        double &bl = baseline[static_cast<size_t>(c.r)][i];
        bl = std::max(bl, idepth[static_cast<size_t>(c.r)][i] * distance);
        valid[static_cast<size_t>(c.r)][i]++;
        inliers[static_cast<size_t>(c.r)][i]++;
      }
    }
    ResidualTable &rt = *w.frames[static_cast<size_t>(c.r)]->residuals[w.frames[static_cast<size_t>(c.t)]->id];
    rt.status.upload(c.status.data(), c.status.size(), 0, st);
    rt.cand.upload(c.cand.data(), c.cand.size(), 0, st);
    rt.energy.upload(c.energy.data(), c.energy.size(), 0, st);
  }
  for (int r = 0; r < F; ++r) {
    HostFrame &f = *w.frames[static_cast<size_t>(r)];
    bool any_conn = false;
    for (const Conn &c : conns) any_conn = any_conn || c.r == r;
    for (int i = 0; i < f.n; ++i) {
      uint8_t &fl = flags[static_cast<size_t>(r)][static_cast<size_t>(i)];
      if (fl & kFlagMarginalized) continue;
      if (valid[static_cast<size_t>(r)][static_cast<size_t>(i)] < 1) fl |= kFlagOutlier;
    }
    (void)any_conn;
    f.dflags.upload(flags[static_cast<size_t>(r)].data(), static_cast<size_t>(f.n), 0, st);
    f.relative_baseline.upload(baseline[static_cast<size_t>(r)].data(), static_cast<size_t>(f.n), 0, st);
    std::vector<int32_t> cur(static_cast<size_t>(f.n));
    f.n_inliers.download(cur.data(), cur.size(), 0, st);
    w.sr.sync();
    for (int i = 0; i < f.n; ++i)
      if (!(flags[static_cast<size_t>(r)][static_cast<size_t>(i)] & kFlagMarginalized)) cur[static_cast<size_t>(i)] = inliers[static_cast<size_t>(r)][static_cast<size_t>(i)];
    f.n_inliers.upload(cur.data(), cur.size(), 0, st);
    w.sr.sync();
    f.flags.resize(static_cast<size_t>(f.n));
    for (int c = 0; c < f.n; ++c) f.flags[static_cast<size_t>(c)] = flags[static_cast<size_t>(r)][static_cast<size_t>(f.internalOf(c))];
  }
  w.sr.sync();
}

bool estimateUncertaintyEnqueue(W &w, bool force_state) {
  prepareDevice(w);
  if (w.fej()) firstEstimate(w);
  w.begun = true;
  stageLinearize(w, false, false, true);
  const int K = w.K();
  const size_t kk = static_cast<size_t>(K) * K;
  const bool want_state = force_state || (w.host_stale && !w.state_dirty);
  const size_t bytes = 2 * kk * sizeof(double) + sizeof(WindowState);
  reserveGeometric(w.h_uncertainty, bytes);
  const hipEvent_t ready = w.uncertainty_ready.get(hipEventDisableTiming);
  double *Hpp = static_cast<double *>(w.h_uncertainty.get()), *Hsc = Hpp + kk;
  w.d_Hpp.download(Hpp, 2 * kk, 0, w.sr.stream);
  if (want_state) HIP_CHECK(hipMemcpyAsync(Hsc + kk, w.d_state.ptr, sizeof(WindowState), hipMemcpyDeviceToHost, w.sr.stream));
  HIP_CHECK(hipEventRecord(ready, w.sr.stream));
  return want_state;
}

void estimateUncertaintyHost(W &w, bool want_state);

void estimateUncertainty(W &w) {
  const bool want_state = estimateUncertaintyEnqueue(w, false);
  estimateUncertaintyHost(w, want_state);
}
// ... 2029 lines not shown
```

### dsopp_amd/csrc/pba_solve_combined.hpp

```cpp
#pragma once
#include "pba_solve_kernels.hpp"

namespace dsopp_hip {

struct SolveCombArgs {
  const FrameDev *frames;
  WindowState *st;
  PairConst *pc;
  const double *comb;
  int comb_copies = 1;
  int comb_copy_first = 0, comb_copy_stride = 0;
  const double *Hm, *bm;
  const double *HmPacked = nullptr;
  double *step;
  LmControl *ctrl;
  double lambda;
  double affine_reg[2];
  double fixed_reg;
  double energy_marginalized;
  int F;
  int fej;
  int use_marginal;
  long long *dbg_stamps;
  const LmControl *dec_in = nullptr;
  const double *dec_scalars = nullptr;
  const SchurBlock *dec_table = nullptr;
  int dec_blocks = 0;
  int dec_groups = 0;
  LmParams dec_prm;
  unsigned *bs_ticket = nullptr;
  double *bs_hand = nullptr;
  double *bs_hand_next = nullptr;
  int bs_parity = 0;
  int dec_chunks = 0;
  unsigned bs_ticket_base = 0;
  int *bs_fault = nullptr;
};
__host__ __device__ inline double kHandOverSentinel() {
  union {
    unsigned long long u;
    double d;
  } c;
  c.u = 0x7FF8D50FF00DBEEFull;
  return c.d;
}
constexpr int kMaxCombCopies = 4;
#define SC_STAMP(i) do { if (kStamps && a.dbg_stamps && tid == 0) a.dbg_stamps[i] = wall_clock64(); } while (0)

__device__ __forceinline__ void combBlockDecode(int b, int &bi, int &bj) {
  int r = static_cast<int>((__fsqrt_rn(8.0f * static_cast<float>(b) + 1.0f) - 1.0f) * 0.5f);
  if ((r + 1) * (r + 2) / 2 <= b) ++r;
  if (r * (r + 1) / 2 > b) --r;
  bi = r;
  bj = b - r * (r + 1) / 2;
}

template <int THREADS, int COPIES = 1>
__global__ void __launch_bounds__(THREADS, 1) solveCombinedKernel(unsigned *bs_ticket_p, double *bs_hand_next_p, const LmControl *dec_in_p,
                                                                  const double *dec_scalars_p, const double *comb_p, const FrameDev *frames_p,
                                                                  WindowState *st_p, int F_p, SolveCombArgs a) {
  extern __shared__ __attribute__((aligned(16))) char smem_raw[];
  const int F = F_p, K = kBlk * F;
  const int N = K + 1;
  const int ld = N + 1;
  double *A = reinterpret_cast<double *>(smem_raw);
  double *pv = A + N * ld;
  double *xs = pv + K;
  double *Linv = xs + K + 16;
  double *epsl = Linv + 36 * kMaxFrames;
  double *stpl = epsl + K;
  double *ab0l = stpl + K;
  const int tid = threadIdx.x;
  const int wave = tid >> 6, lane = tid & 63;
  const long long sc_t_entry = (kStamps && a.dbg_stamps) ? wall_clock64() : 0;

  int c_active = 1, c_relin = 0;
  double lam = a.lambda;
  const bool decides = dec_in_p != nullptr;
  double dec_eps = 0, dec_step = 0;
  int dec_accept = 0;
  const bool ticketed = bs_ticket_p != nullptr;
  unsigned ticket_raw = 0;
  if (ticketed && tid == 0) {
    auto tp = glb(bs_ticket_p);
    asm volatile("" : "+v"(tp));
    ticket_raw = __hip_atomic_fetch_add(tp, 1u, __ATOMIC_RELAXED, __HIP_MEMORY_SCOPE_AGENT);
  }
  if (ticketed && tid < kBlk * kMaxFrames) bs_hand_next_p[tid] = kHandOverSentinel();
  const void DSOPP_CONSTANT *any_words = (const void DSOPP_CONSTANT *)__builtin_amdgcn_kernarg_segment_ptr();
  const LmControl DSOPP_CONSTANT *cin_src = dec_in_p ? (const LmControl DSOPP_CONSTANT *)dec_in_p : (const LmControl DSOPP_CONSTANT *)any_words;
  static_assert(sizeof(a) >= sizeof(LmControl) && sizeof(a) >= 4 * sizeof(double), "the argument block stands in for an absent control block / scalar block");
  static_assert(sizeof(LmControl) == 6 * sizeof(double) + 8 * sizeof(int), "LmControl changed: extend the scalar copy below");
  LmControl cin;
  cin.lambda = cin_src->lambda;
  cin.energy = cin_src->energy;
  cin.cand_prior = cin_src->cand_prior;
  cin.idepth_sq = cin_src->idepth_sq;
  cin.frame_state_sq = cin_src->frame_state_sq;
  cin.frame_step_sq = cin_src->frame_step_sq;
  cin.n_valid = cin_src->n_valid;
  cin.converged = cin_src->converged;
  cin.active = cin_src->active;
  cin.linear_system_valid = cin_src->linear_system_valid;
  cin.iteration = cin_src->iteration;
  cin.need_final_setup = cin_src->need_final_setup;
  cin.pending = cin_src->pending;
  cin.relin = cin_src->relin;
  const double DSOPP_CONSTANT *t_src = dec_scalars_p ? (const double DSOPP_CONSTANT *)dec_scalars_p : (const double DSOPP_CONSTANT *)any_words;
  double t_early[4] = {t_src[0], t_src[1], t_src[2], t_src[3]};
  asm volatile("" : "+s"(cin.lambda), "+s"(cin.energy), "+s"(cin.cand_prior), "+s"(cin.idepth_sq), "+s"(cin.frame_state_sq), "+s"(cin.frame_step_sq),
               "+s"(cin.n_valid), "+s"(cin.converged), "+s"(cin.active), "+s"(cin.linear_system_valid), "+s"(cin.iteration),
               "+s"(cin.need_final_setup), "+s"(cin.pending), "+s"(cin.relin), "+s"(t_early[0]), "+s"(t_early[1]), "+s"(t_early[2]), "+s"(t_early[3])
               : "s"(a.pc), "s"(a.Hm), "s"(a.bm), "s"(a.HmPacked), "s"(a.step), "s"(a.ctrl), "s"(a.fej), "s"(a.use_marginal), "s"(a.dec_table),
               "s"(a.dec_blocks), "s"(a.dec_groups), "s"(a.bs_hand), "s"(a.bs_parity), "s"(a.dec_chunks), "s"(a.bs_ticket_base), "s"(a.comb_copies),
               "s"(a.comb_copy_first), "s"(a.comb_copy_stride), "s"(a.lambda), "s"(a.affine_reg[0]), "s"(a.affine_reg[1]), "s"(a.fixed_reg),
               "s"(a.energy_marginalized));
  __shared__ unsigned s_vblock;
  bool main_wg = ticketed || blockIdx.x == 0;
  struct {
    int valid;
    Rigid T0;
    double fxr, fyr, cxr, cyr, fxt, fyt, cxt, cyt, exposure_r, exposure_t;
  } pp;
  pp.valid = 0;
  const bool fast_refresh = a.fej != 0;
  auto requestPairInputs = [&] {
    if (fast_refresh && tid < F * F) {
      const int r = tid / F, t = tid - F * (tid / F);
      const PairConst &P = a.pc[r * kMaxFrames + t];
      pp.valid = P.valid;
#pragma unroll
      for (int i = 0; i < 3; ++i) {
#pragma unroll
        for (int j = 0; j < 3; ++j) pp.T0.R[3 * i + j] = P.T0rel[4 * i + j];
        pp.T0.t[i] = P.T0rel[4 * i + 3];
      }
      const FrameDev &fr = frames_p[r];
      const FrameDev &ft = frames_p[t];
      pp.fxr = fr.fx;
      pp.fyr = fr.fy;
      pp.cxr = fr.cx;
      pp.cyr = fr.cy;
      pp.fxt = ft.fx;
      pp.fyt = ft.fy;
      pp.cxt = ft.cx;
      pp.cyt = ft.cy;
      pp.exposure_r = fr.exposure;
      pp.exposure_t = ft.exposure;
    }
  };
  double eps_c = 0, ab0_c = 0, rhs_c = 0, bm_c = 0;
  int fixed_c = 0, tomarg_c = 0;
  if (main_wg && tid < K) {
    const int f = tid >> 3, i = tid & 7;
    if (!decides) eps_c = st_p->eps[f][i];
    if (decides) {
      dec_eps = st_p->eps[f][i];
      dec_step = st_p->step[f][i];
    }
    fixed_c = frames_p[f].fixed;
    tomarg_c = frames_p[f].to_marginalize;
    ab0_c = st_p->ab0[f][i < 6 ? 0 : i - 6];
    rhs_c = comb_p[combBlockCount(F) * 64 + tid];
    if (COPIES > 1) {
      for (int cp = 1; cp < a.comb_copies; ++cp)
        rhs_c += comb_p[a.comb_copy_first + static_cast<size_t>(cp - 1) * a.comb_copy_stride + combBlockCount(F) * 64 + tid];
    }
    if (a.use_marginal) bm_c = a.bm[tid];
  }
  const int pc = tid - 64;
  const bool prior_thread = main_wg && pc >= 0 && pc < K;
  double ab0_p = 0, bm_p = 0;
  auto requestTailInputs = [&] {
    if (prior_thread) {
      ab0_p = st_p->ab0[pc >> 3][(pc & 7) < 6 ? 0 : (pc & 7) - 6];
      if (a.use_marginal) bm_p = a.bm[pc];
    }
  };
  if (!ticketed) requestTailInputs();
  const int n_entries = combBlockCount(F) * 64;
  constexpr int kBatch = THREADS >= 512 ? 6 : 8;
  double hv[kBatch], hm[kBatch];
  auto loadBatch = [&](int base) {
#pragma unroll
    for (int u = 0; u < kBatch; ++u) {
      const int e = base + tid + THREADS * u;
      hv[u] = comb_p[min(e, n_entries - 1)];
      hm[u] = 0;
    }
    if (COPIES > 1) {
      double hc[COPIES > 1 ? COPIES - 1 : 1][kBatch];
#pragma unroll
      for (int cp = 1; cp < COPIES; ++cp) {
        const double *cpy = comb_p + a.comb_copy_first + static_cast<size_t>(cp - 1) * a.comb_copy_stride;
#pragma unroll
        for (int u = 0; u < kBatch; ++u) hc[cp - 1][u] = 0;
        if (cp < a.comb_copies) {
#pragma unroll
          for (int u = 0; u < kBatch; ++u) hc[cp - 1][u] = cpy[min(base + tid + THREADS * u, n_entries - 1)];
        }
      }
#pragma unroll
      for (int cp = 1; cp < COPIES; ++cp)
#pragma unroll
        for (int u = 0; u < kBatch; ++u) hv[u] += hc[cp - 1][u];
    }
    if (a.use_marginal) {
#pragma unroll
      for (int u = 0; u < kBatch; ++u) hm[u] = a.HmPacked[min(base + tid + THREADS * u, n_entries - 1)];
    }
  };
  if (main_wg) loadBatch(0);
  if (decides) {
    __shared__ LmControl s_dec_out;
    __shared__ int s_dec_accept, s_dec_proceed;
    double t[4] = {0, 0, 0, 0};
    if (a.dec_groups) {
      __shared__ double s_grp[4 * 8];
      if (tid < 32) {
        const int e = tid >> 3, j = tid & 7;
        const auto gsrc = glb(dec_scalars_p);
        double gv[8];
#pragma unroll
        for (int k = 0; k < 8; ++k) gv[k] = gsrc[4 * (8 * j + k) + e];
        asm volatile("" : "+v"(gv[0]), "+v"(gv[1]), "+v"(gv[2]), "+v"(gv[3]), "+v"(gv[4]), "+v"(gv[5]), "+v"(gv[6]), "+v"(gv[7]));
        double sacc = 0;
#pragma unroll
        for (int k = 0; k < 8; ++k) sacc += gv[k];
        s_grp[e * 8 + j] = sacc;
      }
      ldsBarrier();
      if (tid == 0) {
#pragma unroll
        for (int e = 0; e < 4; ++e) {
          double sacc = 0;
#pragma unroll
          for (int j = 0; j < 8; ++j) sacc += s_grp[e * 8 + j];
          t[e] = sacc;
        }
      }
    } else {
      t[0] = t_early[0];
      t[1] = t_early[1];
      t[2] = t_early[2];
      t[3] = t_early[3];
    }
    if (!cin.active) {
      if (tid == 0 && (ticketed ? ticket_raw == a.bs_ticket_base : blockIdx.x == 0)) *a.ctrl = cin;
      return;
    }
    SC_STAMP(8);
    if (tid == 0) {
      LmControl c;
      int accept = 0, proceed = 0;
      lmDecision(cin, t, a.dec_prm, c, accept, proceed);
      s_dec_out = c;
      s_dec_accept = accept;
      s_dec_proceed = proceed;
      s_vblock = ticketed ? ticket_raw - a.bs_ticket_base : blockIdx.x;
    }
    ldsBarrier();
    SC_STAMP(9);
    dec_accept = s_dec_accept;
    const unsigned vblock = s_vblock;
    main_wg = vblock == 0;
    if (vblock > 0) {
      constexpr int LP = THREADS / 4, CPP = LP / kSchurLandmarks;
      static_assert(CPP >= 1, "a pass covers whole chunks");
      const int W = gridDim.x - 1, n_pass = (a.dec_chunks + CPP - 1) / CPP;
      const int sub = tid & 3, grp = tid >> 2, l = grp & (kSchurLandmarks - 1), chunk_in_pass = grp / kSchurLandmarks;
      if (cin.pending) {
        for (int p = static_cast<int>(vblock) - 1; p < n_pass; p += W) {
          const int chunk = p * CPP + chunk_in_pass;
          if (chunk >= a.dec_chunks) continue;
          const SchurBlock &be = a.dec_table[chunk];
          const int i = be.offset + l;
          if (i >= be.n) continue;
#pragma unroll
          for (int h = 0; h < 4; ++h) {
            const int t2 = sub + 4 * h;
            if (t2 < F && be.status[t2] != nullptr && i < be.n_res[t2]) {
              if (dec_accept)
                be.status[t2][i] = be.cand[t2][i];
              else
                be.cand[t2][i] = be.status[t2][i];
            }
          }
          if (sub == 0) {
            if (dec_accept) be.idepth[i] += be.idepth_step[i];
            be.idepth_step[i] = 0;
          }
        }
      }
      if (!ticketed || !s_dec_proceed || s_dec_out.relin) return;
      auto backSubstitute = [&](auto ns_tag) {
      constexpr int NS = decltype(ns_tag)::value;
      constexpr int kPre = THREADS >= 512 ? (NS >= 4 ? 1 : 2) : 2;
      double rows[kPre][NS][kBlk], bdv[kPre], ihv[kPre];
      hbm_f64 *dstp[kPre];
    #pragma unroll
      for (int u = 0; u < kPre; ++u) {
        dstp[u] = nullptr;
        bdv[u] = ihv[u] = 0;
    #pragma unroll
        for (int q = 0; q < NS; ++q)
    #pragma unroll
          for (int c = 0; c < kBlk; ++c) rows[u][q][c] = 0;
      }
      auto fetch = [&](int p, double (&rw)[NS][kBlk], double &bd, double &ih, hbm_f64 *&dst) {
        dst = nullptr;
        const int chunk = p * CPP + chunk_in_pass;
        if (chunk >= a.dec_chunks) return;
        const SchurBlock &be = a.dec_table[chunk];
        const int i = be.offset + l;
        if (i >= be.n) return;
        const uint8_t flg = be.flags[i];
        if (flg & (kFlagMarginalized | kFlagIllConditioned)) return;
        const size_t plane = ublkPlane(be.cap);
        const hbm_f64 *base = be.ublk + static_cast<size_t>(a.bs_parity) * kMaxFrames * plane + static_cast<size_t>(i) * kUblk;
    #pragma unroll
        for (int q = 0; q < NS; ++q) {
          int t = sub + 4 * q;
          asm volatile("" : "+v"(t));
          if (t < F && (t == be.r || ((be.conn_mask >> t) & 1u))) {
    #pragma unroll
            for (int c = 0; c < kBlk; ++c) rw[q][c] = base[t * plane + c];
          }
        }
        bd = be.b_d[i];
        ih = be.inv_hdd[i];
        dst = be.idepth_step + i;
      };
    #pragma unroll
      for (int u = 0; u < kPre; ++u) {
        const int p = static_cast<int>(vblock) - 1 + u * W;
        if (p < n_pass) fetch(p, rows[u], bdv[u], ihv[u], dstp[u]);
      }
      double *stp = reinterpret_cast<double *>(smem_raw);
      __shared__ int s_timed_out;
      if (tid == 0) s_timed_out = 0;
      ldsBarrier();
      if (tid < kBlk * kMaxFrames) {
        double v = 0;
        if (tid < K) {
          const long long t0 = wall_clock64();
          for (;;) {
            v = __hip_atomic_load(a.bs_hand + tid, __ATOMIC_RELAXED, __HIP_MEMORY_SCOPE_AGENT);
            if (__double_as_longlong(v) != __double_as_longlong(kHandOverSentinel())) break;
            __builtin_amdgcn_s_sleep(24);
            if (wall_clock64() - t0 > 200000000ll) {
              s_timed_out = 1;
              if (a.bs_fault) __hip_atomic_store(a.bs_fault, 1, __ATOMIC_RELAXED, __HIP_MEMORY_SCOPE_SYSTEM);
              break;
            }
          }
        }
        stp[tid] = v;
      }
      __syncthreads();
      if (s_timed_out) return;
      const double damp = 1.0 / (1.0 + s_dec_out.lambda);
      auto finish = [&](const double (&rw)[NS][kBlk], double bd, double ih, hbm_f64 *dst) {
        double d = 0;
    #pragma unroll
        for (int q = 0; q < NS; ++q) {
          const double *sq = stp + kBlk * (sub + 4 * q);
    #pragma unroll
          for (int c = 0; c < kBlk; ++c) d += rw[q][c] * sq[c];
        }
        d += dppMove<0xB1>(d);
        d += dppMove<0x4E>(d);
        if (sub == 0 && dst) *dst = -((bd - d) * damp * ih);
      };
    #pragma unroll
      for (int u = 0; u < kPre; ++u) finish(rows[u], bdv[u], ihv[u], dstp[u]);
      for (int p = static_cast<int>(vblock) - 1 + kPre * W; p < n_pass; p += W) {
        double rw[NS][kBlk], bd = 0, ih = 0;
        hbm_f64 *dst = nullptr;
    #pragma unroll
        for (int q = 0; q < NS; ++q)
    #pragma unroll
          for (int c = 0; c < kBlk; ++c) rw[q][c] = 0;
        fetch(p, rw, bd, ih, dst);
        finish(rw, bd, ih, dst);
      }
      };
      if (THREADS < 512)
        backSubstitute(std::integral_constant<int, 2>{});
      else if (F <= 12)
        backSubstitute(std::integral_constant<int, 3>{});
      else
        backSubstitute(std::integral_constant<int, 4>{});
      return;
    }
    if (cin.pending && tid < K) {
      if (dec_accept) {
        dec_eps += dec_step;
        st_p->eps[tid >> 3][tid & 7] = dec_eps;
      }
      st_p->step[tid >> 3][tid & 7] = 0;
    }
    if (tid == 64) *a.ctrl = s_dec_out;
    if (!s_dec_proceed) return;
    c_active = 1;
    c_relin = s_dec_out.relin;
    lam = s_dec_out.lambda;
  } else if (a.ctrl) {
    c_active = a.ctrl->active;
    c_relin = a.ctrl->relin;
    lam = a.ctrl->lambda;
  }
  if (decides) eps_c = dec_eps;
  SC_STAMP(0);
  if (kStamps && a.dbg_stamps && tid == 0) a.dbg_stamps[7] = sc_t_entry;
  asm volatile("" : "+v"(fixed_c), "+v"(tomarg_c), "+v"(c_active), "+v"(c_relin));
  int prior_kind = 0;
  double pd_c = 0;
  if (tid < K) {
    if (!tomarg_c) prior_kind = fixed_c ? 1 : ((tid & 7) >= 6 ? 2 : 0);
    pd_c = prior_kind == 1 ? a.fixed_reg : (prior_kind == 2 ? ((tid & 7) == 6 ? a.affine_reg[0] : a.affine_reg[1]) : 0.0);
    xs[tid] = eps_c;
    epsl[tid] = eps_c;
    Linv[tid] = pd_c;
    if ((tid & 7) >= 6) ab0l[2 * (tid >> 3) + (tid & 7) - 6] = ab0_c;
  }
  ldsBarrier();
  SC_STAMP(10);
  if (!c_active || c_relin) return;
  const double *prior_diag = Linv;
  const int in_row = (tid >> 3) & 7, in_col = tid & 7;
  double *const A_thr = A + in_row * ld + in_col;
  auto storeBatch = [&](int base) {
    int blk = __builtin_amdgcn_readfirstlane((base + tid) >> 6);
    int bi, bj;
    combBlockDecode(blk, bi, bj);
    bi = __builtin_amdgcn_readfirstlane(bi);
    bj = __builtin_amdgcn_readfirstlane(bj);
    const int n_blocks = n_entries >> 6;
#pragma unroll
    for (int u = 0; u < kBatch; ++u) {
      if (blk < n_blocks) {
        const int blk_off = __builtin_amdgcn_readfirstlane(8 * bi * ld + 8 * bj);
        const double v = hv[u] + hm[u];
        if (bi != bj) {
          A_thr[blk_off] = v;
        } else if (in_col <= in_row) {
          double vd = v;
          if (in_row == in_col) {
            const int row = 8 * bi + in_row;
            vd += prior_diag[row] * (1.0 + lam);
            pv[row] = vd + 10.0;
          }
          A_thr[blk_off] = vd;
        }
      }
      blk += THREADS / 64;
      bj += THREADS / 64;
      while (bj > bi) {
        bj -= bi + 1;
        ++bi;
      }
    }
  };
  storeBatch(0);
  for (int base = kBatch * THREADS; base < n_entries; base += kBatch * THREADS) {
    loadBatch(base);
    storeBatch(base);
  }
  SC_STAMP(11);
  if (tid < K) {
    double v = rhs_c;
    if (prior_kind == 1)
      v += a.fixed_reg * eps_c;
    else if (prior_kind == 2)
      v += ((tid & 7) == 6 ? a.affine_reg[0] : a.affine_reg[1]) * (ab0_c + eps_c);
    if (a.use_marginal) {
      double s = 0;
      for (int k = 0; k < K; ++k) s += a.Hm[tid * K + k] * xs[k];
      v += bm_c + s;
    }
    A[K * ld + tid] = v;
  }
  if (tid == 0) A[K * ld + K] = 0;
  ldsBarrier();
  SC_STAMP(1);
  if (main_wg) requestPairInputs();

  choleskyAugmented<THREADS>(A, pv, Linv, F, tid, a.dbg_stamps);
  SC_STAMP(2);
  if (ticketed) requestTailInputs();
  if (wave == 0) {
    backSubstituteWave(A, Linv, xs, F, lane);
    SC_STAMP(6);
  }
  __syncthreads();
  if (tid < K) {
    const double x = xs[tid];
    stpl[tid] = -x;
    if (a.bs_hand) __hip_atomic_store(a.bs_hand + tid, x, __ATOMIC_RELAXED, __HIP_MEMORY_SCOPE_AGENT);
    a.step[tid] = x;
    st_p->step[tid >> 3][tid & 7] = -x;
  }
  SC_STAMP(3);
  double part = 0, nstate = 0, nstep = 0;
  auto priorMath = [&] {
    if (!a.ctrl || !prior_thread) return;
    const double xc = epsl[pc] + stpl[pc];
    if (a.use_marginal) {
      double sacc = 0;
      for (int k = 0; k < K; ++k) sacc += a.Hm[pc * K + k] * (epsl[k] + stpl[k]);
      part += bm_p * xc + 0.5 * xc * sacc;
    }
    if ((pc & 7) >= 6) {
      const double ab = ab0_p + xc;
      part += 0.5 * ab * ((pc & 7) == 6 ? a.affine_reg[0] : a.affine_reg[1]) * ab;
    }
    nstate = epsl[pc] * epsl[pc] + ((pc & 7) >= 6 ? ab0_p * ab0_p : 0.0);
    nstep = stpl[pc] * stpl[pc];
  };
  if (fast_refresh) {
    ldsBarrier();
    Rigid *E = reinterpret_cast<Rigid *>(A);
    if (tid < 2 * F) {
      const int f = tid < F ? tid : tid - F;
      const double sign = tid < F ? 1.0 : -1.0;
      double xi[6];
#pragma unroll
      for (int i = 0; i < 6; ++i) xi[i] = sign * (epsl[kBlk * f + i] + stpl[kBlk * f + i]);
      E[tid] = rigidExp(xi);
    }
    ldsBarrier();
    asm volatile("" : "+v"(pp.valid));
    if (tid < F * F && pp.valid) {
      const int r = tid / F, t = tid - F * (tid / F);
      PairConst &P = a.pc[r * kMaxFrames + t];
      const Rigid T_tr = rigidMul(E[F + t], rigidMul(pp.T0, E[r]));
      const double ifx = 1.0 / pp.fxr, ify = 1.0 / pp.fyr;
      const double k02 = -pp.cxr * ifx, k12 = -pp.cyr * ify;
      double U[12];
#pragma unroll
      for (int i = 0; i < 3; ++i) {
        U[4 * i + 0] = T_tr.R[3 * i + 0] * ifx;
        U[4 * i + 1] = T_tr.R[3 * i + 1] * ify;
        U[4 * i + 2] = T_tr.R[3 * i + 0] * k02 + T_tr.R[3 * i + 1] * k12 + T_tr.R[3 * i + 2];
        U[4 * i + 3] = T_tr.t[i];
      }
#pragma unroll
      for (int j = 0; j < 4; ++j) {
        P.M[0 + j] = pp.fxt * U[0 + j] + pp.cxt * U[8 + j];
        P.M[4 + j] = pp.fyt * U[4 + j] + pp.cyt * U[8 + j];
        P.M[8 + j] = U[8 + j];
      }
      const double a_r = ab0l[2 * r] + epsl[kBlk * r + 6] + stpl[kBlk * r + 6];
      const double a_t = ab0l[2 * t] + epsl[kBlk * t + 6] + stpl[kBlk * t + 6];
      P.s = (pp.exposure_t / pp.exposure_r) * exp(a_t - a_r);
      P.b_t = ab0l[2 * t + 1] + epsl[kBlk * t + 7] + stpl[kBlk * t + 7];
      P.b_r = ab0l[2 * r + 1] + epsl[kBlk * r + 7] + stpl[kBlk * r + 7];
    }
    priorMath();
  } else {
    ldsBarrier();
    priorMath();
  }
  SC_STAMP(4);
  if (a.ctrl && K <= 64) {
    if (wave == 1) {
      part = waveSum(part);
      nstate = waveSum(nstate);
      nstep = waveSum(nstep);
      if (tid == 64) {
        a.ctrl->cand_prior = a.energy_marginalized + part;
        a.ctrl->frame_state_sq = nstate;
        a.ctrl->frame_step_sq = nstep;
        a.ctrl->pending = 1;
      }
    }
  } else if (a.ctrl) {
    part = waveSum(part);
    nstate = waveSum(nstate);
    nstep = waveSum(nstep);
    ldsBarrier();
    if ((tid & 63) == 0) {
      xs[tid >> 6] = part;
      xs[THREADS / 64 + (tid >> 6)] = nstate;
      xs[2 * (THREADS / 64) + (tid >> 6)] = nstep;
    }
    ldsBarrier();
    if (tid == 64) {
      constexpr int kWaves = THREADS / 64;
      double total = a.energy_marginalized, s_state = 0, s_step = 0;
      for (int w = 0; w < kWaves; ++w) {
        total += xs[w];
        s_state += xs[kWaves + w];
        s_step += xs[2 * kWaves + w];
      }
      a.ctrl->cand_prior = total;
      a.ctrl->frame_state_sq = s_state;
      a.ctrl->frame_step_sq = s_step;
      a.ctrl->pending = 1;
    }
  }
  SC_STAMP(5);
}

}
```

### dsopp_amd/csrc/pba_solve_kernels.hpp

```cpp
#pragma once
#include <cstddef>
#include <type_traits>
#include "pba_kernels.hpp"

namespace dsopp_hip {


struct LmParams {
  double function_tolerance, parameter_tolerance;
  double decrease_on_accept, increase_on_reject;
  double lambda0;
  int max_iterations, min_iterations;
  int force_accept;
  int use_reduced_scalars;
};

constexpr int kSchurLandmarks = 64;
constexpr int kSchurThreads = 512;
constexpr int kPairBlk = 144;

__host__ __device__ inline int schurRowStride(int Kp) {
  return ((Kp + 15) / 32) * 32 + 16;
}

__device__ inline void derivePairBlocks(const double *__restrict__ G , const PairConst &P, double *__restrict__ out ,
                                        double *lds , int lane) {
  const int i = lane >> 3, j = lane & 7;
  double gt;
  if (j < 6) {
    gt = 0;
#pragma unroll
    for (int k = 0; k < 6; ++k) gt += G[symIdx(i, k)] * P.Adj[6 * k + j];
  } else if (j == 6) {
    gt = G[symIdx(i, 6)];
  } else {
    gt = G[symIdx(i, 7)] * P.s0;
  }
  lds[lane] = gt;
  out[64 + lane] = gt;
  __builtin_amdgcn_s_waitcnt(0);
  __builtin_amdgcn_wave_barrier();
  double tgt;
  if (i < 6) {
    tgt = 0;
#pragma unroll
    for (int k = 0; k < 6; ++k) tgt += P.Adj[6 * k + i] * lds[8 * k + j];
  } else if (i == 6) {
    tgt = lds[48 + j];
  } else {
    tgt = P.s0 * lds[56 + j];
  }
  out[lane] = tgt;
  if (lane < 8) {
    const double *q = G + 36;
    double s;
    if (lane < 6) {
      s = 0;
#pragma unroll
      for (int k = 0; k < 6; ++k) s += P.Adj[6 * k + lane] * q[k];
    } else if (lane == 6) {
      s = q[6];
    } else {
      s = P.s0 * q[7];
    }
    out[128 + lane] = s;
  }
}

__host__ __device__ constexpr int combBlockIndex(int bi, int bj) { return bi * (bi + 1) / 2 + bj; }
__host__ __device__ constexpr int combBlockCount(int F) { return F * (F + 1) / 2; }
__device__ __forceinline__ int combIndex(int row, int col) { return combBlockIndex(row >> 3, col >> 3) * 64 + ((row & 7) << 3) + (col & 7); }

struct ReduceSchurArgs {
  const FrameDev *frames;
  const PairConst *pc;
  const SchurBlock *schur_table;
  const double *partials;
  const int *pair_first_block, *pair_num_blocks;
  double *Hpp, *bpp;
  double *Hsc, *bsc;
  const LmControl *ctrl;
  int F;
  int n_schur_blocks;
  int for_marginalized;
  int ublk_parity;
  LmControl *ctrl_out;
  WindowState *st;
  const double *scalars;
  int n_sweep_blocks;
  int total_blocks;
  double *scalars_out;
  int scalars_out_groups = 0;
  double *comb;
  int comb_copies = 1;
  int comb_copy_first = 0, comb_copy_stride = 0;
  double comb_lambda;
  LmParams prm;
  long long *dbg;
  LmControl *ctrl_host = nullptr;
};
#define RS_STAMP(i) do { if (kStamps && a.dbg && threadIdx.x == 0 && blockIdx.x == 1) a.dbg[i] = wall_clock64(); } while (0)

using f64x4 = __attribute__((ext_vector_type(4))) double;

constexpr int kScalarGroups = 64;

struct ApplyRegs {
  uint8_t *p_status[2], *p_cand[2];
  uint8_t v_status[2], v_cand[2];
  double *p_idepth, *p_istep;
  double v_idepth, v_istep;
  double st_eps, st_step;
  const LmControl *out;
  int accept, pending, publish;
};

__device__ inline void applyDecision(const ReduceSchurArgs &a, const ApplyRegs &ar) {
  const int tid = threadIdx.x;
  if (ar.pending) {
#pragma unroll
    for (int h = 0; h < 2; ++h) {
      if (ar.p_status[h] == nullptr) continue;
      if (ar.accept)
        *ar.p_status[h] = ar.v_cand[h];
      else
        *ar.p_cand[h] = ar.v_status[h];
    }
    if (ar.p_idepth != nullptr) {
      if (ar.accept) *ar.p_idepth = ar.v_idepth + ar.v_istep;
      *ar.p_istep = 0;
    }
    if (blockIdx.x == 0 && tid < kBlk * a.F) {
      const int f = tid >> 3, c = tid & 7;
      if (ar.accept) a.st->eps[f][c] = ar.st_eps + ar.st_step;
      a.st->step[f][c] = 0;
    }
  }
  if (ar.publish && blockIdx.x == 0 && tid == 0) {
    *a.ctrl_out = *ar.out;
    if (a.ctrl_host) *a.ctrl_host = *ar.out;
  }
}

__device__ inline void lmDecision(const LmControl &cin, const double (&t)[4], const LmParams &prm, LmControl &c, int &accept, int &proceed) {
  c = cin;
  accept = 0;
  proceed = 0;
  const double eval_energy = t[0] + cin.cand_prior;
  const int n_valid = static_cast<int>(t[1] + 0.5);
  if (!cin.pending) {
    if (cin.relin) {
      c.relin = 0;
      proceed = 1;
    } else {
      c.idepth_sq = t[2];
      c.energy = eval_energy;
      c.n_valid = n_valid;
      c.active = (prm.max_iterations > 0 && n_valid > 0) ? 1 : 0;
      proceed = c.active;
    }
  } else {
    c.iteration = cin.iteration + 1;
    c.pending = 0;
    if (n_valid == 0) {
      c.active = 0;
      c.need_final_setup = 1;
    } else {
      if (fabs(cin.energy - eval_energy) / cin.energy < prm.function_tolerance) c.converged = 1;
      if (eval_energy < cin.energy || (prm.force_accept && cin.iteration < prm.min_iterations)) {
        accept = 1;
        const double state_sq = cin.frame_state_sq + cin.idepth_sq, step_sq = cin.frame_step_sq + t[2];
        if (step_sq < prm.parameter_tolerance * (state_sq + prm.parameter_tolerance)) c.converged = 1;
        c.energy = eval_energy;
        c.n_valid = n_valid;
        c.lambda = cin.lambda / prm.decrease_on_accept;
        c.idepth_sq = cin.idepth_sq + 2.0 * t[3] + t[2];
        c.need_final_setup = 0;
        proceed = 1;
      } else {
        c.need_final_setup = 1;
        if (prm.force_accept) {
          c.active = 0;
        } else {
          c.lambda = cin.lambda * prm.increase_on_reject;
          c.relin = 1;
        }
      }
      if (c.converged || c.iteration >= prm.max_iterations) c.active = 0;
    }
    if (!c.active) proceed = 0;
  }
}

__device__ inline bool fusedDecideApply(const ReduceSchurArgs &a, double *lds, long long *dbg_out, ApplyRegs &ar) {
  __shared__ LmControl s_out;
  __shared__ int s_accept, s_proceed;
  __shared__ long long s_dbg[2];
  const int tid = threadIdx.x;
  const LmControl cin = *a.ctrl;
  ar.out = &s_out;
  ar.pending = 0;
  ar.accept = 0;
  ar.publish = 0;
  const bool is_schur = static_cast<int>(blockIdx.x) < a.n_schur_blocks;
  uint8_t *p_status[2] = {nullptr, nullptr}, *p_cand[2] = {nullptr, nullptr};
  uint8_t v_status[2] = {0, 0}, v_cand[2] = {0, 0};
  double *p_idepth = nullptr, *p_istep = nullptr;
  double v_idepth = 0, v_istep = 0;
  if (is_schur) {
    const SchurBlock &be = a.schur_table[blockIdx.x];
    const int l = tid >> 3, sub = tid & 7;
    const int i = be.offset + l;
    if (i < be.n) {
#pragma unroll
      for (int h = 0; h < 2; ++h) {
        const int t = sub + 8 * h;
        if (t < a.F && be.status[t] != nullptr && i < be.n_res[t]) {
          p_status[h] = be.status[t] + i;
          p_cand[h] = be.cand[t] + i;
          v_status[h] = *p_status[h];
          v_cand[h] = *p_cand[h];
        }
      }
      if (sub == 0) {
        p_idepth = be.idepth + i;
        p_istep = be.idepth_step + i;
        v_idepth = *p_idepth;
        v_istep = *p_istep;
      }
    }
  }
  double st_eps = 0, st_step = 0;
  if (blockIdx.x == 0 && tid < kBlk * a.F) {
    const int f = tid >> 3, c = tid & 7;
    st_eps = a.st->eps[f][c];
    st_step = a.st->step[f][c];
  }
  double v[4] = {0, 0, 0, 0};
  if (a.prm.use_reduced_scalars == 2) {
    if (tid < kScalarGroups) {
      const double *p = a.scalars + 4 * tid;
      v[0] = p[0];
      v[1] = p[1];
      v[2] = p[2];
      v[3] = p[3];
    }
  } else if (a.prm.use_reduced_scalars) {
    if (tid == 0) {
      v[0] = a.scalars[0];
      v[1] = a.scalars[1];
      v[2] = a.scalars[2];
      v[3] = a.scalars[3];
    }
  } else {
    for (int b = tid; b < a.n_sweep_blocks; b += kSchurThreads) {
      const double *p = a.partials + static_cast<size_t>(b) * kPartial;
      v[0] += p[44];
      v[1] += p[45];
      v[2] += p[46];
      v[3] += p[47];
    }
  }
  if (!cin.active) {
    if (blockIdx.x == 0 && tid == 0) {
      *a.ctrl_out = cin;
      if (a.ctrl_host) *a.ctrl_host = cin;
    }
    return false;
  }
  const bool direct = a.prm.use_reduced_scalars == 1;
  constexpr int RS = kSchurThreads + 2;
  static_assert(kSchurThreads == 512, "reduction tree below assumes 512 threads");
  double *l2 = lds + 6 * RS;
  double *l3 = l2 + 6 * 64;
  if (!direct) {
#pragma unroll
    for (int e = 0; e < 4; ++e) lds[e * RS + tid] = v[e];
    ldsBarrier();
    if (kStamps && a.dbg && tid == 0) s_dbg[0] = wall_clock64();
    if (tid < 4 * 64) {
      const int e = tid >> 6, j = tid & 63;
      double s = 0;
#pragma unroll
      for (int k = 0; k < 8; ++k) s += lds[e * RS + 8 * j + k];
      l2[e * 64 + j] = s;
    }
    ldsBarrier();
    if (tid < 4 * 8) {
      const int e = tid >> 3, j = tid & 7;
      double s = 0;
#pragma unroll
      for (int k = 0; k < 8; ++k) s += l2[e * 64 + 8 * j + k];
      l3[e * 8 + j] = s;
    }
    ldsBarrier();
  }
  if (tid == 0) {
    double t[4];
#pragma unroll
    for (int e = 0; e < 4; ++e) {
      double s = 0;
      if (direct) {
        s = v[e];
      } else {
#pragma unroll
        for (int k = 0; k < 8; ++k) s += l3[e * 8 + k];
      }
      t[e] = s;
    }
    LmControl c;
    int accept = 0, proceed = 0;
    lmDecision(cin, t, a.prm, c, accept, proceed);
    s_accept = accept;
    s_proceed = proceed;
    s_out = c;
  }
  ldsBarrier();
  if (kStamps && a.dbg && tid == 0) s_dbg[1] = wall_clock64();
  if (kStamps && a.dbg && tid == 0) { dbg_out[0] = s_dbg[0]; dbg_out[1] = s_dbg[1]; }
  ar.accept = s_accept;
  ar.pending = cin.pending;
  ar.publish = 1;
#pragma unroll
  for (int h = 0; h < 2; ++h) {
    ar.p_status[h] = p_status[h];
    ar.p_cand[h] = p_cand[h];
    ar.v_status[h] = v_status[h];
    ar.v_cand[h] = v_cand[h];
  }
  ar.p_idepth = p_idepth;
  ar.p_istep = p_istep;
  ar.v_idepth = v_idepth;
  ar.v_istep = v_istep;
  ar.st_eps = st_eps;
  ar.st_step = st_step;
  return s_proceed != 0;
}

__global__ void __launch_bounds__(kSchurThreads) reduceSchurKernel(const LmControl *ctrl_p, const SchurBlock *table_p, const PairConst *pc_p,
                                                                   const double *partials_p, const int *pair_first_p, const int *pair_num_p,
                                                                   int n_schur_blocks_p, int F_p, ReduceSchurArgs a) {
  extern __shared__ __attribute__((aligned(16))) char smem_raw[];
  a.ctrl = ctrl_p;
  a.schur_table = table_p;
  a.pc = pc_p;
  a.partials = partials_p;
  a.pair_first_block = pair_first_p;
  a.pair_num_blocks = pair_num_p;
  a.n_schur_blocks = n_schur_blocks_p;
  a.F = F_p;
  const long long rs_t0 = (kStamps && a.dbg) ? wall_clock64() : 0;
  long long rs_dbg[2] = {0, 0};
  static_assert(sizeof(ReduceSchurArgs) >= sizeof(LmControl), "the argument block stands in for an absent control block");
  static_assert(sizeof(ReduceSchurArgs) >= offsetof(SchurBlock, flags) + sizeof(SchurBlock::flags) && sizeof(ReduceSchurArgs) >= offsetof(SchurBlock, ublk) + sizeof(SchurBlock::ublk),
                "the argument block stands in for the head of an absent Schur descriptor");
  const void DSOPP_CONSTANT *any_words = (const void DSOPP_CONSTANT *)__builtin_amdgcn_kernarg_segment_ptr();
  const LmControl DSOPP_CONSTANT *cp = ctrl_p ? (const LmControl DSOPP_CONSTANT *)ctrl_p : (const LmControl DSOPP_CONSTANT *)any_words;
  int c_active = cp->active, c_lsv = cp->linear_system_valid;
  double comb_lam = cp->lambda;
  struct SchurHead {
    int r, offset, n, cap;
  } hd = {0, 0, 0, 0};
  unsigned hd_conn = 0;
  decltype(SchurBlock::ublk) hd_ublk = nullptr;
  decltype(SchurBlock::flags) hd_flags = nullptr;
  {
    const SchurBlock DSOPP_CONSTANT *dp =
        n_schur_blocks_p > 0 ? (const SchurBlock DSOPP_CONSTANT *)table_p + min(static_cast<int>(blockIdx.x), n_schur_blocks_p - 1)
                             : (const SchurBlock DSOPP_CONSTANT *)any_words;
    const SchurBlock DSOPP_CONSTANT &d = *dp;
    hd = {d.r, d.offset, d.n, d.cap};
    hd_conn = d.conn_mask;
    hd_ublk = d.ublk;
    hd_flags = d.flags;
  }
  asm volatile("" ::"s"(a.frames), "s"(a.Hpp), "s"(a.bpp), "s"(a.Hsc), "s"(a.bsc), "s"(a.for_marginalized), "s"(a.ublk_parity), "s"(a.ctrl_out),
               "s"(a.st), "s"(a.scalars), "s"(a.n_sweep_blocks), "s"(a.scalars_out), "s"(a.scalars_out_groups), "s"(a.comb), "s"(a.comb_lambda), "s"(a.comb_copies),
               "s"(a.comb_copy_first), "s"(a.comb_copy_stride));
  asm volatile("" : "+s"(hd.r), "+s"(hd.offset), "+s"(hd.n), "+s"(hd.cap), "+s"(hd_conn), "+s"(hd_ublk), "+s"(hd_flags), "+s"(c_active), "+s"(c_lsv),
               "+s"(comb_lam));
  if (!ctrl_p) {
    c_active = 1;
    c_lsv = 0;
    comb_lam = a.comb_lambda;
  }
  if (n_schur_blocks_p <= 0) {
    hd = {0, 0, 0, 0};
    hd_conn = 0;
    hd_ublk = nullptr;
    hd_flags = nullptr;
  }
  if (!c_active || c_lsv) return;
  const int F = a.F, K = kBlk * F;
  double *const comb_w = (a.comb && a.comb_copies > 1 && (blockIdx.x % a.comb_copies) != 0)
                             ? a.comb + a.comb_copy_first + static_cast<size_t>(blockIdx.x % a.comb_copies - 1) * a.comb_copy_stride
                             : a.comb;
  if (a.scalars_out && static_cast<int>(blockIdx.x) == a.n_schur_blocks + F * F) {
    double *lds = reinterpret_cast<double *>(smem_raw);
    double v[4] = {0, 0, 0, 0};
    for (int b = threadIdx.x; b < a.n_sweep_blocks; b += kSchurThreads) {
      const double *p = a.partials + static_cast<size_t>(b) * kPartial + 44;
      v[0] += p[0];
      v[1] += p[1];
      v[2] += p[2];
      v[3] += p[3];
    }
#pragma unroll
    for (int e = 0; e < 4; ++e) lds[e * (kSchurThreads + 2) + threadIdx.x] = v[e];
    __syncthreads();
    if (threadIdx.x < 4) {
      double sacc = 0;
      for (int j = 0; j < kSchurThreads; ++j) sacc += lds[threadIdx.x * (kSchurThreads + 2) + j];
      a.scalars_out[threadIdx.x] = sacc;
    } else if (static_cast<int>(threadIdx.x) < 4 * a.scalars_out_groups) {
      a.scalars_out[threadIdx.x] = 0;
    }
    return;
  }
  if (static_cast<int>(blockIdx.x) >= a.n_schur_blocks) {
    const int p = blockIdx.x - a.n_schur_blocks;
    const int r = p / F, t = p % F, pi = r * kMaxFrames + t;
    const int lane = threadIdx.x & 63, wave = threadIdx.x >> 6;
    const PairConst &P = a.pc[pi];
    const int valid = P.valid;
    double *lds = reinterpret_cast<double *>(smem_raw);
    double *wsum = lds + 48 + 64 + kPairBlk;
    {
      double sw = 0;
      if (valid && lane < 44) {
        const int first = a.pair_first_block[pi], cnt = a.pair_num_blocks[pi];
        const double *src = a.partials + static_cast<size_t>(first) * kPartial + lane;
        int b = wave;
        for (; b + 8 < cnt; b += 16) sw += src[static_cast<size_t>(b) * kPartial] + src[static_cast<size_t>(b + 8) * kPartial];
        if (b < cnt) sw += src[static_cast<size_t>(b) * kPartial];
      }
      if (lane < 48) wsum[wave * 48 + lane] = sw;
    }
    ldsBarrier();
    if (threadIdx.x >= 64 || !valid) return;
    double s = 0;
    if (lane < 44) {
#pragma unroll
      for (int w = 0; w < kSchurThreads / 64; ++w) s += wsum[w * 48 + lane];
    }
    if (lane < 48) lds[lane] = s;
    __builtin_amdgcn_s_waitcnt(0);
    __builtin_amdgcn_wave_barrier();
    double *drv = lds + 48 + 64;
    derivePairBlocks(lds, P, drv, lds + 48, lane);
    __builtin_amdgcn_s_waitcnt(0);
    __builtin_amdgcn_wave_barrier();
    const int i = lane >> 3, j = lane & 7;
    if (a.comb) {
      const double dl = i == j ? 1.0 + comb_lam : 1.0;
      atomicAdd(&comb_w[combBlockIndex(r, r) * 64 + lane], dl * drv[lane]);
      atomicAdd(&comb_w[combBlockIndex(t, t) * 64 + lane], dl * lds[symIdx(i, j)]);
      if (r > t)
        atomicAdd(&comb_w[combBlockIndex(r, t) * 64 + lane], -drv[64 + 8 * j + i]);
      else
        atomicAdd(&comb_w[combBlockIndex(t, r) * 64 + lane], -drv[64 + lane]);
      if (lane < 8) {
        double *rhs = comb_w + combBlockCount(F) * 64;
        atomicAdd(&rhs[kBlk * r + lane], drv[128 + lane]);
        atomicAdd(&rhs[kBlk * t + lane], -lds[36 + lane]);
      }
      return;
    }
    atomicAdd(&a.Hpp[(kBlk * r + i) * K + kBlk * r + j], drv[lane]);
    atomicAdd(&a.Hpp[(kBlk * t + i) * K + kBlk * t + j], lds[symIdx(i, j)]);
    atomicAdd(&a.Hpp[(kBlk * r + i) * K + kBlk * t + j], -drv[64 + 8 * j + i]);
    atomicAdd(&a.Hpp[(kBlk * t + i) * K + kBlk * r + j], -drv[64 + lane]);
    if (lane < 8) {
      atomicAdd(&a.bpp[kBlk * r + lane], drv[128 + lane]);
      atomicAdd(&a.bpp[kBlk * t + lane], -lds[36 + lane]);
    }
    return;
  }
  const double comb_sc = -1.0 / (1.0 + comb_lam);
  const int Kp = (K + 15) & ~15;
  const int stride = schurRowStride(Kp);
  double *hrow = reinterpret_cast<double *>(smem_raw);
  double *wgt = hrow + kSchurLandmarks * stride;
  double *wbd = wgt + kSchurLandmarks;
  const SchurBlock &be = a.schur_table[blockIdx.x];
  const int r = hd.r;
  const bool bd_in_pad = K < Kp;
  if (kStamps && a.dbg && threadIdx.x == 0 && blockIdx.x == 1) { a.dbg[0] = rs_t0; a.dbg[6] = rs_dbg[0]; a.dbg[7] = rs_dbg[1]; }
  RS_STAMP(1);
  const int l = threadIdx.x >> 3, sub = threadIdx.x & 7;
  const int i = hd.offset + l;
  const unsigned conn = hd_conn & ~(1u << r);
  const size_t plane = ublkPlane(hd.cap);
  const double *ubase = hd_ublk + static_cast<size_t>(a.ublk_parity) * kMaxFrames * plane + static_cast<size_t>(i) * kUblk;
  bool take = false;
  uint8_t flg = 0;
  if (i < hd.n) {
    flg = hd_flags[i];
    take = a.for_marginalized ? (flg & kFlagToMarginalize) != 0 : (flg & kFlagMarginalized) == 0;
  }
  double ht[kUblk];
#pragma unroll
  for (int c = 0; c < kUblk; ++c) ht[c] = 0;
  const bool first = i < hd.n && sub < F && ((conn >> sub) & 1u);
  if (first) {
    const double *src = ubase + sub * plane;
#pragma unroll
    for (int c = 0; c < kUblk; ++c) ht[c] = src[c];
  }
  double tmv = 0;
  if (static_cast<int>(threadIdx.x) < F * 37) {
    const int t = threadIdx.x / 37, c = threadIdx.x - 37 * t;
    const PairConst &P = a.pc[r * kMaxFrames + t];
    tmv = c < 36 ? P.Adj[c] : P.s0;
  }
  for (int idx = threadIdx.x; idx < kSchurLandmarks * stride; idx += kSchurThreads) hrow[idx] = 0;
  double *Tm = wbd + kSchurLandmarks;
  if (static_cast<int>(threadIdx.x) < F * 37) {
    const int t = threadIdx.x / 37, c = threadIdx.x - 37 * t;
    Tm[t * 40 + c] = tmv;
  }
  for (int e = threadIdx.x + kSchurThreads; e < F * 37; e += kSchurThreads) {
    const int t = e / 37, c = e - 37 * t;
    const PairConst &P = a.pc[r * kMaxFrames + t];
    Tm[t * 40 + c] = c < 36 ? P.Adj[c] : P.s0;
  }
  ldsBarrier();
  RS_STAMP(2);
  {
    double hr[kBlk];
#pragma unroll
    for (int c = 0; c < kBlk; ++c) hr[c] = 0;
    double hdd = 0, bd = 0;
    double *row = hrow + l * stride;
    if (take) {
      for (int t = sub; t < F; t += 8) {
        if (!((conn >> t) & 1u)) continue;
        if (t != sub) {
          const double *src = ubase + t * plane;
#pragma unroll
          for (int c = 0; c < kUblk; ++c) ht[c] = src[c];
        }
        const double *Tt = Tm + t * 40;
#pragma unroll
        for (int c = 0; c < kBlk; ++c) row[kBlk * t + c] = ht[c];
        hdd += ht[8];
        bd += ht[9];
#pragma unroll
        for (int c = 0; c < 6; ++c) {
          double s = 0;
#pragma unroll
          for (int k = 0; k < 6; ++k) s += Tt[6 * k + c] * ht[k];
          hr[c] -= s;
        }
        hr[6] -= ht[6];
        hr[7] -= Tt[36] * ht[7];
      }
    }
#pragma unroll
    for (int c = 0; c < kBlk; ++c) hr[c] = sum8(hr[c]);
    hdd = sum8(hdd);
    bd = sum8(bd);
    if (sub == 0) {
      double inv = 0, ibd = 0;
      if (take) {
        double *dst = const_cast<double *>(ubase) + r * plane;
#pragma unroll
        for (int c = 0; c < kBlk; ++c) {
          row[kBlk * r + c] = hr[c];
          dst[c] = hr[c];
        }
        be.b_d[i] = bd;
        const double kIdepthNullSpaceThreshold = 1e-15;
        if (hdd > kIdepthNullSpaceThreshold) {
          if (a.for_marginalized && be.fixed) hdd += 1e8;
          inv = 1.0 / hdd;
          be.inv_hdd[i] = inv;
          flg &= static_cast<uint8_t>(~kFlagIllConditioned);
          ibd = inv * bd;
        } else {
          flg |= kFlagIllConditioned;
        }
        be.flags[i] = flg;
      }
      wgt[l] = inv;
      wbd[l] = ibd;
      if (bd_in_pad && take) row[K] = bd;
    }
  }
  ldsBarrier();
  RS_STAMP(3);
  {
    const int lane = threadIdx.x & 63, wave = threadIdx.x >> 6;
    const int nt = Kp >> 4;
    const int n_tiles = nt * (nt + 1) / 2;
    const int li = lane & 15, lk = lane >> 4;
    for (int tile = wave; tile < n_tiles; tile += kSchurThreads / 64) {
      int ti = 0, rem = tile;
      while (rem >= nt - ti) {
        rem -= nt - ti;
        ++ti;
      }
      const int tj = ti + rem;
      f64x4 acc = {0, 0, 0, 0};
      const double *pa = hrow + lk * stride + 16 * ti + li;
      const double *pb = hrow + lk * stride + 16 * tj + li;
      constexpr int kSteps = kSchurLandmarks / 4;
      double av[kSteps], bv[kSteps], wv[kSteps];
#pragma unroll
      for (int q = 0; q < kSteps; ++q) {
        wv[q] = wgt[4 * q + lk];
        av[q] = pa[4 * q * stride];
        bv[q] = pb[4 * q * stride];
      }
#pragma unroll
      for (int q = 0; q < kSteps; ++q) acc = __builtin_amdgcn_mfma_f64_16x16x4f64(wv[q] * av[q], bv[q], acc, 0, 0, 0);
#pragma unroll
      for (int reg = 0; reg < 4; ++reg) {
        const int row = 16 * ti + lk + 4 * reg, col = 16 * tj + li;
        const double v = acc[reg];
        if (a.comb) {
          const double sv = v * comb_sc;
          if (row < K && col < K && col >= row && v != 0) atomicAdd(&comb_w[combIndex(col, row)], sv);
          if (bd_in_pad && row < K && col == K && v != 0) atomicAdd(&comb_w[combBlockCount(F) * 64 + row], sv);
          continue;
        }
        if (row < K && col < K && col >= row && v != 0) atomicAdd(&a.Hsc[row * K + col], v);
        if (bd_in_pad && row < K && col == K && v != 0) atomicAdd(&a.bsc[row], v);
      }
    }
    RS_STAMP(4);
    for (int c = threadIdx.x; c < (bd_in_pad ? 0 : K); c += kSchurThreads) {
      double s = 0;
#pragma unroll 1
      for (int ll = 0; ll < kSchurLandmarks; ++ll) s += wbd[ll] * hrow[ll * stride + c];
      if (s != 0) {
        if (a.comb)
          atomicAdd(&comb_w[combBlockCount(F) * 64 + c], s * comb_sc);
        else
          atomicAdd(&a.bsc[c], s);
      }
    }
    RS_STAMP(5);
  }
}

__global__ void __launch_bounds__(kSchurThreads) decideApplyKernel(ReduceSchurArgs a) {
  extern __shared__ __attribute__((aligned(16))) char smem_raw[];
  long long dbg_unused[2] = {0, 0};
  ApplyRegs ar;
  ar.pending = 0;
  ar.publish = 0;
  fusedDecideApply(a, reinterpret_cast<double *>(smem_raw), dbg_unused, ar);
  applyDecision(a, ar);
}

__global__ void clearSchurKernel(double *buf, int n, const LmControl *ctrl) {
  if (ctrl && (!ctrl->active || ctrl->linear_system_valid)) return;
  const int i = blockIdx.x * blockDim.x + threadIdx.x;
  if (i < n) buf[i] = 0;
}

constexpr int kSolveThreads = 256;

struct SolveArgs {
  const FrameDev *frames;
  WindowState *st;
  PairConst *pc;
  const double *Hpp_raw, *bpp_raw;
  double *Hsc;
  const double *bsc;
  double *Hpp_out, *bpp_out;
  double *Hsc_copy = nullptr;
  const double *Hm, *bm;
  double *step;
  double lambda;
  double affine_reg[2];
  double fixed_reg;
  double energy_marginalized;
  int F;
  int fej;
  int do_solve;
  int store_system;
  int add_priors;
  int use_marginal;
};

__device__ inline double priorEnergyBlock(const SolveArgs &a, bool with_step, double *lds , int tid) {
  const int F = a.F, K = kBlk * F;
  for (int c = tid; c < K; c += kSolveThreads) lds[c] = a.st->eps[c >> 3][c & 7] + (with_step ? a.st->step[c >> 3][c & 7] : 0.0);
  __syncthreads();
  double part = 0;
  for (int c = tid; c < K; c += kSolveThreads) {
    if (a.use_marginal) {
      double s = 0;
      for (int k = 0; k < K; ++k) s += a.Hm[c * K + k] * lds[k];
      part += a.bm[c] * lds[c] + 0.5 * lds[c] * s;
    }
    if ((c & 7) >= 6) {
      const double ab = a.st->ab0[c >> 3][(c & 7) - 6] + lds[c];
      part += 0.5 * ab * a.affine_reg[(c & 7) - 6] * ab;
    }
  }
  part = waveSum(part);
  __syncthreads();
  if ((tid & 63) == 0) lds[K + (tid >> 6)] = part;
  __syncthreads();
  double total = a.energy_marginalized;
  for (int w = 0; w < kSolveThreads / 64; ++w) total += lds[K + w];
  __syncthreads();
  return total;
}

__host__ __device__ constexpr int lowIdx(int i, int j) { return i * (i + 1) / 2 + j; }

__device__ __forceinline__ double readLane(double v, int src_lane) {
  const int lo = __builtin_amdgcn_readlane(__double2loint(v), src_lane);
  const int hi = __builtin_amdgcn_readlane(__double2hiint(v), src_lane);
  return __hiloint2double(hi, lo);
}

template <int THREADS>
__device__ __forceinline__ void choleskyAugmented(double *A, const double *pv, double *Linv, int F, int tid, long long *stamps) {
  const int K = kBlk * F;
  const int N = K + 1;
  const int ld = N + 1;
  const int wave = tid >> 6, lane = tid & 63;
  auto factorAndPanel = [&](int kb) {
    const int k0 = kb * kBlk;
    const int row = k0 + lane;
    const bool valid = row < N;
    double c[kBlk], invd[kBlk], lj[28];
    {
      const double *src = A + (valid ? row : k0) * ld + k0;
#pragma unroll
      for (int j = 0; j < kBlk; ++j) c[j] = src[j];
    }
    double guard[kBlk];
#pragma unroll
    for (int k = 0; k < kBlk; ++k) guard[k] = 1e-30 * pv[min(k0 + k, K - 1)];
    int e = 0;
    auto rsqrtRefined = [](double d) {
      const double hd = 0.5 * d;
      double inv = __builtin_amdgcn_rsq(d);
      inv = fma(inv, fma(-hd * inv, inv, 0.5), inv);
      inv = fma(inv, fma(-hd * inv, inv, 0.5), inv);
      return inv;
    };
#pragma unroll
    for (int k = 0; k < kBlk; ++k) {
      const double d = readLane(c[k], k);
      const bool okp = d > guard[k];
      double inv = rsqrtRefined(d);
      inv = okp ? inv : 0.0;
      invd[k] = inv;
      const double l = c[k] * inv;
      c[k] = l;
#pragma unroll
      for (int j = k + 1; j < kBlk; ++j) {
        const double ljk = readLane(l, j);
        lj[e++] = ljk;
        c[j] -= l * ljk;
      }
    }
    if (valid) {
      double *dst = A + row * ld + k0;
#pragma unroll
      for (int j = 0; j < kBlk; ++j)
        if (lane >= kBlk || j <= lane) dst[j] = c[j];
    }
    for (int r2 = row + 64; r2 < N; r2 += 64) {
      double v[kBlk];
#pragma unroll
      for (int j = 0; j < kBlk; ++j) v[j] = A[r2 * ld + k0 + j];
      int e2 = 0;
#pragma unroll
      for (int k = 0; k < kBlk; ++k) {
        v[k] *= invd[k];
#pragma unroll
        for (int j = k + 1; j < kBlk; ++j) v[j] -= v[k] * lj[e2++];
      }
#pragma unroll
      for (int j = 0; j < kBlk; ++j) A[r2 * ld + k0 + j] = v[j];
    }
    if (lane == 0) {
#pragma unroll
      for (int cidx = 0; cidx < kBlk; ++cidx) Linv[kb * 36 + lowIdx(cidx, cidx)] = invd[cidx];
    }
  };
  long long cs_acc[4] = {0, 0, 0, 0}, cs_t = (kStamps && stamps) ? wall_clock64() : 0;
  auto csMark = [&](int slot) {
    if (kStamps && stamps) {
      const long long now = wall_clock64();
      cs_acc[slot] += now - cs_t;
      cs_t = now;
    }
  };
  if (wave == 0) factorAndPanel(0);
  ldsBarrier();
  csMark(2);
  for (int kb = 0; kb < F; ++kb) {
    const int k0 = kb * kBlk, k1 = k0 + kBlk, k2 = k1 + kBlk;
    if (kb + 1 < F) {
      const int n_el = (N - k1) * kBlk;
      for (int e = tid; e < n_el; e += THREADS) {
        const int row = k1 + (e >> 3), col = k1 + (e & 7);
        if (col > row) continue;
        const double *li = A + row * ld + k0, *lj = A + col * ld + k0;
        double sacc = 0;
#pragma unroll
        for (int c = 0; c < kBlk; ++c) sacc += li[c] * lj[c];
        A[row * ld + col] -= sacc;
      }
    }
    csMark(0);
    ldsBarrier();
    csMark(1);
    if (wave == 0) {
      if (kb + 1 < F) factorAndPanel(kb + 1);
      csMark(2);
    } else {
      const int t = tid - 64, tr = t >> 4, tc = t & 15;
      for (int row = k2 + tr; row < N; row += (THREADS - 64) / 16) {
        const double *li = A + row * ld + k0;
        double lic[kBlk];
#pragma unroll
        for (int c = 0; c < kBlk; ++c) lic[c] = li[c];
        for (int col = k2 + tc; col <= row; col += 16) {
          const double *lj = A + col * ld + k0;
          double sacc = 0;
#pragma unroll
          for (int c = 0; c < kBlk; ++c) sacc += lic[c] * lj[c];
          A[row * ld + col] -= sacc;
        }
      }
    }
    ldsBarrier();
    csMark(3);
  }
  if (kStamps && stamps && tid == 0) {
    for (int q = 0; q < 4; ++q) stamps[12 + q] = cs_acc[q];
  }
}

__device__ __forceinline__ void backSubstituteWave(const double *A, const double *Linv, double *xs, int F, int lane) {
  const int K = kBlk * F, ld = K + 2;
  auto run = [&](auto two_tag) {
    constexpr bool TWO = decltype(two_tag)::value;
    const int j0 = lane, j1 = lane + 64;
    double y0 = j0 < K ? A[K * ld + j0] : 0.0, y1 = (TWO && j1 < K) ? A[K * ld + j1] : 0.0;
    const double gi0 = j0 < K ? Linv[(j0 >> 3) * 36 + lowIdx(j0 & 7, j0 & 7)] : 0.0;
    const double gi1 = (TWO && j1 < K) ? Linv[(j1 >> 3) * 36 + lowIdx(j1 & 7, j1 & 7)] : 0.0;
    double g0[kBlk], g1[kBlk], n0[kBlk], n1[kBlk];
    auto loadBlock = [&](int kb, double *o0, double *o1) {
#pragma unroll
      for (int c = 0; c < kBlk; ++c) {
        o0[c] = A[(kb * kBlk + c) * ld + j0];
        if (TWO) o1[c] = j1 < K ? A[(kb * kBlk + c) * ld + j1] : 0.0;
      }
    };
    auto sweepBlocks = [&](auto upper_tag, int kb_from, int kb_to) {
      constexpr bool UPPER = decltype(upper_tag)::value;
      for (int kb = kb_from; kb >= kb_to; --kb) {
        if (kb > 0) {
#pragma unroll
          for (int c = 0; c < kBlk; ++c) {
            n0[c] = A[((kb - 1) * kBlk + c) * ld + j0];
            if (UPPER) n1[c] = j1 < K ? A[((kb - 1) * kBlk + c) * ld + j1] : 0.0;
          }
        }
        double xo[kBlk];
#pragma unroll
        for (int c = kBlk - 1; c >= 0; --c) {
          const int k = kb * kBlk + c;
          const double xk = UPPER ? readLane(y1 * gi1, k & 63) : readLane(y0 * gi0, k);
          xo[c] = xk;
          y0 -= g0[c] * xk;
          if (UPPER) y1 -= g1[c] * xk;
        }
        if (lane == 0) {
#pragma unroll
          for (int c = 0; c < kBlk; ++c) xs[kb * kBlk + c] = xo[c];
        }
#pragma unroll
        for (int c = 0; c < kBlk; ++c) {
          g0[c] = n0[c];
          if (UPPER) g1[c] = n1[c];
        }
      }
    };
    loadBlock(F - 1, g0, g1);
    if (TWO) {
      sweepBlocks(std::true_type{}, F - 1, 8);
      sweepBlocks(std::false_type{}, 7, 0);
    } else {
      sweepBlocks(std::false_type{}, F - 1, 0);
    }
  };
  if (K > 64)
    run(std::true_type{});
  else
    run(std::false_type{});
}

__global__ void __launch_bounds__(kSolveThreads, 1) assembleSolveKernel(SolveArgs a) {
  extern __shared__ __attribute__((aligned(16))) char smem_raw[];
  const int F = a.F, K = kBlk * F;
  const int N = K + 1;
  const int ld = N + 1;
  double *A = reinterpret_cast<double *>(smem_raw);
  double *pv = A + N * ld;
  double *xs = pv + K;
  double *Linv = xs + K + 16;
  const int tid = threadIdx.x;
  const double lam = a.lambda;
  double eps_c = 0, ab0_c = 0, bpp_c = 0, bsc_c = 0, bm_c = 0;
  int fixed_c = 0, tomarg_c = 0;
  if (tid < K) {
    const int f = tid >> 3, i = tid & 7;
    eps_c = a.st->eps[f][i];
    fixed_c = a.frames[f].fixed;
    tomarg_c = a.frames[f].to_marginalize;
    ab0_c = a.st->ab0[f][i < 6 ? 0 : i - 6];
    bpp_c = a.bpp_raw[tid];
    bsc_c = a.bsc[tid];
    if (a.use_marginal) bm_c = a.bm[tid];
  }
  double *prior_diag = Linv;
  const int tile_r = tid >> 4, tile_c = tid & 15;
  const int nt = (K + 15) >> 4, n_tiles = nt * (nt + 1) / 2;
  constexpr int kTileBatch = 12;
  double hp[kTileBatch], hs[kTileBatch], hm[kTileBatch];
  int rows[kTileBatch], cols[kTileBatch];
  auto loadBatch = [&](int base) {
#pragma unroll
    for (int u = 0; u < kTileBatch; ++u) {
      int tile = base + u, tr0 = 0;
      while (tile >= tr0 + 1) {
        tile -= tr0 + 1;
        ++tr0;
      }
// ... 327 lines not shown
```

Measured before the change: 26490 GN iterations/s.

## Replace atomic combined-system accumulation with per-block partials summed in solve kernel

```diff
diff --git a/dsopp_amd/csrc/pba.hip b/dsopp_amd/csrc/pba.hip
--- a/dsopp_amd/csrc/pba.hip
+++ b/dsopp_amd/csrc/pba.hip
@@ -108,9 +108,14 @@
   }
   size_t reduceCount() const { return 2 * (static_cast<size_t>(K()) * K() + K()); }
   size_t combCount() const { return static_cast<size_t>(combBlockCount(F())) * 64 + static_cast<size_t>(K()); }
-  int comb_copies_active = 1;
-  size_t combCopyFirst() const { return (combCount() + 4 * kScalarGroups + 8 + 1) & ~static_cast<size_t>(1); }
-  size_t combCopyStride() const { return (combCount() + 1) & ~static_cast<size_t>(1); }
+  bool combSummed() const { return !twoStage() && !allreduce; }
+  size_t combPartStride() const { return (combCount() + 1) & ~static_cast<size_t>(1); }
+  int combParts() const { return opt.optimize_idepths ? n_schur_blocks : 0; }
+  DeviceBuffer<double> d_comb_parts, d_comb_pairs;
+  DeviceMem<unsigned> d_comb_hand;
+  static constexpr size_t kCombHand = static_cast<size_t>(combBlockCount(kMaxFrames)) * 64 + static_cast<size_t>(kBlk) * kMaxFrames;
+  size_t comb_armed_count = 0;
+  unsigned comb_seq = 0, comb_claim_base = 0;
   int n_sweep_blocks = 0, n_schur_blocks = 0;
   bool topology_dirty = true;
   bool frames_dirty = false;
@@ -719,7 +724,7 @@
   const size_t KK = static_cast<size_t>(kBlk * kMaxFrames);
   w.d_Hpp.reserve(2 * KK * KK, 0, st);
   w.d_bpp.reserve(KK, 0, st);
-  w.d_reduce.reserve(2 * (KK * KK + KK) + 8 + 4 * kScalarGroups + 16 + static_cast<size_t>(kMaxCombCopies - 1) * (static_cast<size_t>(combBlockCount(kMaxFrames)) * 64 + KK + 2), 0, st);
+  w.d_reduce.reserve(2 * (KK * KK + KK) + 8 + 4 * kScalarGroups + 16, 0, st);
   w.d_Hm.reserve(KK * KK, 0, st);
   w.d_bm.reserve(KK, 0, st);
   w.d_step.reserve(KK, 0, st);
@@ -840,8 +845,7 @@
   prm.ctrl = ctrl;
   prm.clear_buf = lin ? w.d_reduce.ptr : nullptr;
   prm.clear_count = static_cast<int>(ex.combined ? w.combCount() + 4 : w.reduceCount());
-  if (ex.combined && w.comb_copies_active > 1)
-    prm.clear_count = static_cast<int>(w.combCopyFirst() + (w.comb_copies_active - 1) * w.combCopyStride());
+  if (ex.combined && w.combSummed()) prm.clear_buf = nullptr;
   prm.step = w.d_step.ptr;
   prm.lambda = lambda;
   prm.F = w.F();
@@ -958,10 +962,12 @@
   const size_t reduce_count = combined ? w.combCount() : w.reduceCount();
   a.comb = combined ? w.d_reduce.ptr : nullptr;
   a.comb_lambda = fused ? fused->comb_lambda : 0.0;
-  if (combined && mode == ReduceMode::kAccumulateOnly && w.comb_copies_active > 1) {
-    a.comb_copies = w.comb_copies_active;
-    a.comb_copy_first = static_cast<int>(w.combCopyFirst());
-    a.comb_copy_stride = static_cast<int>(w.combCopyStride());
+  if (combined && mode == ReduceMode::kAccumulateOnly && w.combSummed()) {
+    w.d_comb_parts.reserve(std::max<size_t>(1, static_cast<size_t>(a.n_schur_blocks)) * w.combPartStride(), 0, st);
+    w.d_comb_pairs.reserve(static_cast<size_t>(kMaxFrames) * kMaxFrames * kPairSlot, 0, st);
+    a.comb_parts = w.d_comb_parts.ptr;
+    a.comb_pairs = w.d_comb_pairs.ptr;
+    a.comb_part_stride = static_cast<int>(w.combPartStride());
   }
   a.scalars = mode == ReduceMode::kDecideOnly ? w.d_reduce.ptr + reduce_count : w.d_scalars.ptr;
   a.n_sweep_blocks = w.n_sweep_blocks;
@@ -1107,10 +1113,24 @@
   return n;
 }
 
+__global__ void armCombHandOverKernel(unsigned *claim, double *hand, int n) {
+  const int i = blockIdx.x * blockDim.x + threadIdx.x;
+  if (i == 0) *claim = 0;
+  if (i < n) hand[i] = kHandOverSentinel();
+}
+
+void armCombHandOver(W &w) {
+  const int n = static_cast<int>(2 * W::kCombHand);
+  armCombHandOverKernel<<<(n + 255) / 256, 256, 0, w.sr.stream>>>(w.d_comb_hand.get(), reinterpret_cast<double *>(reinterpret_cast<char *>(w.d_comb_hand.get()) + 16), n);
+  HIP_CHECK(hipGetLastError());
+  w.comb_seq = 0;
+  w.comb_claim_base = 0;
+  w.comb_armed_count = w.combCount();
+}
+
 void launchSolveCombined(W &w, double lambda, LmControl *ctrl, const LmControl *decide_from = nullptr, const LmParams *decide_prm = nullptr,
                          bool decide_from_groups = false, bool backsub = false, int ublk_parity = 0) {
   ensureDynamicLds(reinterpret_cast<const void *>(solveCombinedKernel<256>), w.sr.device, 150 * 1024);
-  ensureDynamicLds(reinterpret_cast<const void *>(solveCombinedKernel<256, kMaxCombCopies>), w.sr.device, 150 * 1024);
   ensureDynamicLds(reinterpret_cast<const void *>(solveCombinedKernel<512>), w.sr.device, 150 * 1024);
   SolveCombArgs a;
   if (decide_from) {
@@ -1120,6 +1140,8 @@
     a.dec_chunks = w.n_schur_blocks;
     const bool wide = w.F() > 8;
     a.dec_blocks = std::min(wide ? (w.n_schur_blocks + 1) / 2 : w.n_schur_blocks, solveResidentWorkgroups(w, wide) - 1);
+    static const int landmark_wgs_max = std::getenv("DSOPP_HIP_SOLVE_LANDMARK_WGS_MAX") ? std::atoi(std::getenv("DSOPP_HIP_SOLVE_LANDMARK_WGS_MAX")) : 0;
+    if (landmark_wgs_max > 0) a.dec_blocks = std::min(a.dec_blocks, landmark_wgs_max);
     a.dec_groups = decide_from_groups ? kScalarGroups : 0;
     a.dec_prm = *decide_prm;
     if (backsub && a.dec_blocks > 0) {
@@ -1150,10 +1172,36 @@
   a.st = w.d_state.ptr;
   a.pc = w.d_pc.ptr;
   a.comb = w.d_reduce.ptr;
-  if (w.comb_copies_active > 1) {
-    a.comb_copies = w.comb_copies_active;
-    a.comb_copy_first = static_cast<int>(w.combCopyFirst());
-    a.comb_copy_stride = static_cast<int>(w.combCopyStride());
+  if (w.combSummed()) {
+    const int threads = w.F() > 8 ? 512 : 256;
+    w.d_comb_parts.reserve(std::max<size_t>(1, static_cast<size_t>(w.combParts())) * w.combPartStride(), 0, w.sr.stream);
+    w.d_comb_pairs.reserve(static_cast<size_t>(kMaxFrames) * kMaxFrames * kPairSlot, 0, w.sr.stream);
+    if (!w.d_comb_hand) {
+      w.d_comb_hand.alloc(16 + 2 * W::kCombHand * sizeof(double));
+      armCombHandOver(w);
+    } else if (w.comb_armed_count != w.combCount()) {
+      armCombHandOver(w);
+    }
+    if (!w.h_bs_fault) {
+      w.h_bs_fault.reserve(sizeof(int));
+      *w.h_bs_fault.get() = 0;
+    }
+    a.bs_fault = w.h_bs_fault.get();
+    a.comb_parts = w.d_comb_parts.ptr;
+    a.comb_pairs = w.d_comb_pairs.ptr;
+    a.comb_part_stride = static_cast<int>(w.combPartStride());
+    a.comb_n_parts = w.combParts();
+    const int n_terms = a.comb_n_parts + 2 * w.F() - 1;
+    int lg = 6;
+    while (lg > 4 && (n_terms + (threads >> lg) - 1) / (threads >> lg) > 16) --lg;
+    a.comb_slice_log2 = lg;
+    a.comb_per_group = (n_terms + (threads >> lg) - 1) / (threads >> lg);
+    a.comb_n_slices = static_cast<int>((w.combCount() + (size_t(1) << lg) - 1) >> lg);
+    double *hand = reinterpret_cast<double *>(reinterpret_cast<char *>(w.d_comb_hand.get()) + 16);
+    a.comb_claim = w.d_comb_hand.get();
+    a.comb_claim_base = w.comb_claim_base;
+    a.comb_hand = hand + (w.comb_seq & 1u) * W::kCombHand;
+    a.comb_hand_next = hand + ((w.comb_seq + 1) & 1u) * W::kCombHand;
   }
   a.Hm = w.d_Hm.ptr;
   a.HmPacked = w.d_Hm_packed.ptr;
@@ -1174,9 +1222,6 @@
                 if (w.F() > 8)
                   solveCombinedKernel<512><<<1 + a.dec_blocks, 512, solveSmemBytes(w.K()), w.sr.stream>>>(
                       a.bs_ticket, a.bs_hand_next, a.dec_in, a.dec_scalars, a.comb, a.frames, a.st, a.F, a);
-                else if (a.comb_copies > 1)
-                  solveCombinedKernel<256, kMaxCombCopies><<<1 + a.dec_blocks, 256, solveSmemBytes(w.K()), w.sr.stream>>>(
-                      a.bs_ticket, a.bs_hand_next, a.dec_in, a.dec_scalars, a.comb, a.frames, a.st, a.F, a);
                 else
                   solveCombinedKernel<256><<<1 + a.dec_blocks, 256, solveSmemBytes(w.K()), w.sr.stream>>>(
                       a.bs_ticket, a.bs_hand_next, a.dec_in, a.dec_scalars, a.comb, a.frames, a.st, a.F, a);
@@ -1186,6 +1231,10 @@
     w.bs_seq++;
     w.bs_ticket_base += static_cast<unsigned>(1 + a.dec_blocks);
   }
+  if (a.comb_parts) {
+    w.comb_seq++;
+    w.comb_claim_base += static_cast<unsigned>(a.comb_n_slices + 1 + a.dec_blocks);
+  }
   if (!w.fej()) {
     pairSetupKernel<<<1, kMaxFrames * kMaxFrames, 0, w.sr.stream>>>(w.d_frames.ptr, w.d_state.ptr, w.d_pc.ptr, w.F(), 0, nullptr);
     HIP_CHECK(hipGetLastError());
@@ -1195,15 +1244,18 @@
 void checkSolveLaunchFault(W &w) {
   if (!w.h_bs_fault || !*w.h_bs_fault.get()) return;
   *w.h_bs_fault.get() = 0;
-  constexpr size_t kHand = static_cast<size_t>(kBlk) * kMaxFrames;
-  std::vector<double> arm(2 * kHand, kHandOverSentinel());
-  HIP_CHECK(hipMemsetAsync(w.d_bs_flag.get(), 0, 16, w.sr.stream));
-  HIP_CHECK(hipMemcpyAsync(reinterpret_cast<char *>(w.d_bs_flag.get()) + 16, arm.data(), arm.size() * sizeof(double), hipMemcpyHostToDevice, w.sr.stream));
-  HIP_CHECK(hipStreamSynchronize(w.sr.stream));
-  w.bs_seq = 0;
-  w.bs_ticket_base = 0;
-  fail(DSOPP_HIP_ERR_HIP, "a solve launch's landmark workgroups waited 2 s for the pose step (device shared with a kernel that never yields?): "
-                          "the inverse depths of that iteration were not updated, the solve is void");
+  if (w.d_bs_flag) {
+    constexpr size_t kHand = static_cast<size_t>(kBlk) * kMaxFrames;
+    std::vector<double> arm(2 * kHand, kHandOverSentinel());
+    HIP_CHECK(hipMemsetAsync(w.d_bs_flag.get(), 0, 16, w.sr.stream));
+    HIP_CHECK(hipMemcpyAsync(reinterpret_cast<char *>(w.d_bs_flag.get()) + 16, arm.data(), arm.size() * sizeof(double), hipMemcpyHostToDevice, w.sr.stream));
+    HIP_CHECK(hipStreamSynchronize(w.sr.stream));
+    w.bs_seq = 0;
+    w.bs_ticket_base = 0;
+  }
+  if (w.d_comb_hand) armCombHandOver(w);
+  fail(DSOPP_HIP_ERR_HIP, "a solve launch's workgroups waited 2 s for the combined system or the pose step (device shared with a kernel that never "
+                          "yields?): that iteration was not completed, the solve is void");
 }
 
 void launchBacksub(W &w, double lambda, const LmControl *ctrl, int ublk_parity = 0, bool gate_on_pending = false) {
@@ -1388,12 +1440,6 @@
   const int rounds = (w.opt.force_accept ? w.opt.max_iterations : 2 * w.opt.max_iterations) + 1;
   bool result_written_by_kernel = false;
   const bool k3_backsub = w.opt.optimize_idepths && w.n_schur_blocks > 0;
-  static const int comb_copies_min_chunks = std::getenv("DSOPP_HIP_COMB_COPIES_MIN_CHUNKS") ? std::atoi(std::getenv("DSOPP_HIP_COMB_COPIES_MIN_CHUNKS")) : 80;
-  w.comb_copies_active = (!w.twoStage() && !w.allreduce && w.F() <= 7 && w.n_schur_blocks >= comb_copies_min_chunks) ? kMaxCombCopies : 1;
-  struct CopiesReset {
-    W &w;
-    ~CopiesReset() { w.comb_copies_active = 1; }
-  } copies_reset{w};
   for (int r = 0; r < rounds; ++r) {
     LmControl *cin = ctrl + (r & 1), *cout = ctrl + ((r + 1) & 1);
     SweepExtras ex;
diff --git a/dsopp_amd/csrc/pba_solve_combined.hpp b/dsopp_amd/csrc/pba_solve_combined.hpp
--- a/dsopp_amd/csrc/pba_solve_combined.hpp
+++ b/dsopp_amd/csrc/pba_solve_combined.hpp
@@ -8,8 +8,13 @@
   WindowState *st;
   PairConst *pc;
   const double *comb;
-  int comb_copies = 1;
-  int comb_copy_first = 0, comb_copy_stride = 0;
+  const double *comb_parts = nullptr;
+  const double *comb_pairs = nullptr;
+  int comb_part_stride = 0, comb_n_parts = 0;
+  int comb_slice_log2 = 6, comb_per_group = 0, comb_n_slices = 0;
+  unsigned *comb_claim = nullptr;
+  unsigned comb_claim_base = 0;
+  double *comb_hand = nullptr, *comb_hand_next = nullptr;
   const double *Hm, *bm;
   const double *HmPacked = nullptr;
   double *step;
@@ -44,7 +49,6 @@
   c.u = 0x7FF8D50FF00DBEEFull;
   return c.d;
 }
-constexpr int kMaxCombCopies = 4;
 #define SC_STAMP(i) do { if (kStamps && a.dbg_stamps && tid == 0) a.dbg_stamps[i] = wall_clock64(); } while (0)
 
 __device__ __forceinline__ void combBlockDecode(int b, int &bi, int &bj) {
@@ -55,7 +59,7 @@
   bj = b - r * (r + 1) / 2;
 }
 
-template <int THREADS, int COPIES = 1>
+template <int THREADS>
 __global__ void __launch_bounds__(THREADS, 1) solveCombinedKernel(unsigned *bs_ticket_p, double *bs_hand_next_p, const LmControl *dec_in_p,
                                                                   const double *dec_scalars_p, const double *comb_p, const FrameDev *frames_p,
                                                                   WindowState *st_p, int F_p, SolveCombArgs a) {
@@ -87,6 +91,14 @@
     ticket_raw = __hip_atomic_fetch_add(tp, 1u, __ATOMIC_RELAXED, __HIP_MEMORY_SCOPE_AGENT);
   }
   if (ticketed && tid < kBlk * kMaxFrames) bs_hand_next_p[tid] = kHandOverSentinel();
+  const bool summed = a.comb_parts != nullptr;
+  unsigned claim_raw = 0;
+  auto drawClaim = [&] {
+    auto cp = glb(a.comb_claim);
+    asm volatile("" : "+v"(cp));
+    claim_raw = __hip_atomic_fetch_add(cp, 1u, __ATOMIC_RELAXED, __HIP_MEMORY_SCOPE_AGENT);
+  };
+  if (summed && tid == 0) drawClaim();
   const void DSOPP_CONSTANT *any_words = (const void DSOPP_CONSTANT *)__builtin_amdgcn_kernarg_segment_ptr();
   const LmControl DSOPP_CONSTANT *cin_src = dec_in_p ? (const LmControl DSOPP_CONSTANT *)dec_in_p : (const LmControl DSOPP_CONSTANT *)any_words;
   static_assert(sizeof(a) >= sizeof(LmControl) && sizeof(a) >= 4 * sizeof(double), "the argument block stands in for an absent control block / scalar block");
@@ -112,8 +124,9 @@
                "+s"(cin.n_valid), "+s"(cin.converged), "+s"(cin.active), "+s"(cin.linear_system_valid), "+s"(cin.iteration),
                "+s"(cin.need_final_setup), "+s"(cin.pending), "+s"(cin.relin), "+s"(t_early[0]), "+s"(t_early[1]), "+s"(t_early[2]), "+s"(t_early[3])
                : "s"(a.pc), "s"(a.Hm), "s"(a.bm), "s"(a.HmPacked), "s"(a.step), "s"(a.ctrl), "s"(a.fej), "s"(a.use_marginal), "s"(a.dec_table),
-               "s"(a.dec_blocks), "s"(a.dec_groups), "s"(a.bs_hand), "s"(a.bs_parity), "s"(a.dec_chunks), "s"(a.bs_ticket_base), "s"(a.comb_copies),
-               "s"(a.comb_copy_first), "s"(a.comb_copy_stride), "s"(a.lambda), "s"(a.affine_reg[0]), "s"(a.affine_reg[1]), "s"(a.fixed_reg),
+               "s"(a.dec_blocks), "s"(a.dec_groups), "s"(a.bs_hand), "s"(a.bs_parity), "s"(a.dec_chunks), "s"(a.bs_ticket_base), "s"(a.comb_parts),
+               "s"(a.comb_pairs), "s"(a.comb_part_stride), "s"(a.comb_n_parts), "s"(a.comb_slice_log2), "s"(a.comb_per_group), "s"(a.comb_n_slices),
+               "s"(a.comb_claim), "s"(a.comb_claim_base), "s"(a.comb_hand), "s"(a.comb_hand_next), "s"(a.lambda), "s"(a.affine_reg[0]), "s"(a.affine_reg[1]), "s"(a.fixed_reg),
                "s"(a.energy_marginalized));
   __shared__ unsigned s_vblock;
   bool main_wg = ticketed || blockIdx.x == 0;
@@ -161,11 +174,7 @@
     fixed_c = frames_p[f].fixed;
     tomarg_c = frames_p[f].to_marginalize;
     ab0_c = st_p->ab0[f][i < 6 ? 0 : i - 6];
-    rhs_c = comb_p[combBlockCount(F) * 64 + tid];
-    if (COPIES > 1) {
-      for (int cp = 1; cp < a.comb_copies; ++cp)
-        rhs_c += comb_p[a.comb_copy_first + static_cast<size_t>(cp - 1) * a.comb_copy_stride + combBlockCount(F) * 64 + tid];
-    }
+    if (!summed) rhs_c = comb_p[combBlockCount(F) * 64 + tid];
     if (a.use_marginal) bm_c = a.bm[tid];
   }
   const int pc = tid - 64;
@@ -185,32 +194,106 @@
 #pragma unroll
     for (int u = 0; u < kBatch; ++u) {
       const int e = base + tid + THREADS * u;
-      hv[u] = comb_p[min(e, n_entries - 1)];
+      hv[u] = summed ? __hip_atomic_load(glb(a.comb_hand) + min(e, n_entries - 1), __ATOMIC_RELAXED, __HIP_MEMORY_SCOPE_AGENT) : comb_p[min(e, n_entries - 1)];
       hm[u] = 0;
     }
-    if (COPIES > 1) {
-      double hc[COPIES > 1 ? COPIES - 1 : 1][kBatch];
-#pragma unroll
-      for (int cp = 1; cp < COPIES; ++cp) {
-        const double *cpy = comb_p + a.comb_copy_first + static_cast<size_t>(cp - 1) * a.comb_copy_stride;
-#pragma unroll
-        for (int u = 0; u < kBatch; ++u) hc[cp - 1][u] = 0;
-        if (cp < a.comb_copies) {
-#pragma unroll
-          for (int u = 0; u < kBatch; ++u) hc[cp - 1][u] = cpy[min(base + tid + THREADS * u, n_entries - 1)];
-        }
-      }
-#pragma unroll
-      for (int cp = 1; cp < COPIES; ++cp)
-#pragma unroll
-        for (int u = 0; u < kBatch; ++u) hv[u] += hc[cp - 1][u];
-    }
     if (a.use_marginal) {
 #pragma unroll
       for (int u = 0; u < kBatch; ++u) hm[u] = a.HmPacked[min(base + tid + THREADS * u, n_entries - 1)];
     }
   };
-  if (main_wg) loadBatch(0);
+  if (main_wg && !summed) loadBatch(0);
+  __shared__ int s_comb_fault;
+  if (tid == 0) s_comb_fault = 0;
+  auto isArmed = [](double v) { return __double_as_longlong(v) == __double_as_longlong(kHandOverSentinel()); };
+  auto awaitSlot = [&](double &v, int e) {
+    if (!isArmed(v)) return;
+    const long long t0 = wall_clock64();
+    for (;;) {
+      v = __hip_atomic_load(glb(a.comb_hand) + e, __ATOMIC_RELAXED, __HIP_MEMORY_SCOPE_AGENT);
+      if (!isArmed(v)) break;
+      __builtin_amdgcn_s_sleep(4);
+      if (wall_clock64() - t0 > 200000000ll) {
+        s_comb_fault = 1;
+        if (a.bs_fault) __hip_atomic_store(a.bs_fault, 1, __ATOMIC_RELAXED, __HIP_MEMORY_SCOPE_SYSTEM);
+        break;
+      }
+    }
+  };
+  auto awaitBatch = [&](int base) {
+    if (!summed) return;
+#pragma unroll
+    for (int u = 0; u < kBatch; ++u) awaitSlot(hv[u], min(base + tid + THREADS * u, n_entries - 1));
+  };
+  __shared__ unsigned s_claim;
+  __shared__ double s_part[THREADS];
+  auto claimSlices = [&](bool sum) {
+    const int lg = a.comb_slice_log2, ent = tid & ((1 << lg) - 1), grp = tid >> lg;
+    const int n_total = n_entries + K;
+    const auto parts = glb(a.comb_parts);
+    const auto pairs = glb(a.comb_pairs);
+    for (;;) {
+      if (tid == 0) s_claim = claim_raw - a.comb_claim_base;
+      ldsBarrier();
+      const unsigned sl = s_claim;
+      if (sl >= static_cast<unsigned>(a.comb_n_slices)) break;
+      if (tid == 0) drawClaim();
+      const int e = static_cast<int>(sl << lg) + ent, ec = min(e, n_total - 1);
+      const bool live = e < n_total;
+      if (sum) {
+        int kind, fa, fb = 0, idx;
+        if (ec < n_entries) {
+          combBlockDecode(ec >> 6, fa, fb);
+          kind = fa == fb ? 1 : 0;
+          idx = ec & 63;
+        } else {
+          kind = 2;
+          fa = (ec - n_entries) >> 3;
+          idx = (ec - n_entries) & 7;
+        }
+        const int n_terms = a.comb_n_parts + (kind == 0 ? 2 : 2 * F - 1);
+        auto term = [&](int v, int v_end) {
+          const bool ok = v < v_end && v < n_terms;
+          const int k = ok ? v - a.comb_n_parts : 0;
+          int r, t, sec;
+          if (kind == 0) {
+            r = k == 0 ? fb : fa;
+            t = k == 0 ? fa : fb;
+            sec = 128;
+          } else {
+            const bool as_ref = k >= fa && k < fa + F;
+            r = k < fa ? k : (as_ref ? fa : k - F + 1);
+            t = as_ref ? k - fa : fa;
+            sec = kind == 1 ? (as_ref ? 0 : 64) : (as_ref ? 192 : 200);
+          }
+          const bool from_part = ok && v < a.comb_n_parts;
+          const auto src = from_part ? parts + (static_cast<size_t>(v) * a.comb_part_stride + ec)
+                                     : pairs + (static_cast<size_t>(max(r, 0) * F + max(t, 0)) * kPairSlot + sec + idx);
+          const double x = *src;
+          return ok ? x : 0.0;
+        };
+        double acc = 0;
+        const int v0 = grp * a.comb_per_group, v1 = v0 + a.comb_per_group;
+        for (int vb = v0; vb < v1; vb += 8) {
+          double x[8];
+#pragma unroll
+          for (int u = 0; u < 8; ++u) x[u] = term(vb + u, v1);
+          asm volatile("" : "+v"(x[0]), "+v"(x[1]), "+v"(x[2]), "+v"(x[3]), "+v"(x[4]), "+v"(x[5]), "+v"(x[6]), "+v"(x[7]));
+#pragma unroll
+          for (int u = 0; u < 8; ++u) acc += x[u];
+        }
+        s_part[tid] = acc;
+        ldsBarrier();
+        if (grp == 0 && live) {
+          double tot = 0;
+          for (int g = 0; g < (THREADS >> lg); ++g) tot += s_part[(g << lg) + ent];
+          __hip_atomic_store(glb(a.comb_hand) + e, tot, __ATOMIC_RELAXED, __HIP_MEMORY_SCOPE_AGENT);
+        }
+      }
+      if (grp == 0 && live) a.comb_hand_next[e] = kHandOverSentinel();
+      ldsBarrier();
+    }
+  };
   if (decides) {
     __shared__ LmControl s_dec_out;
     __shared__ int s_dec_accept, s_dec_proceed;
@@ -247,6 +330,7 @@
     }
     if (!cin.active) {
       if (tid == 0 && (ticketed ? ticket_raw == a.bs_ticket_base : blockIdx.x == 0)) *a.ctrl = cin;
+      if (summed) claimSlices(false);
       return;
     }
     SC_STAMP(8);
@@ -263,6 +347,7 @@
     SC_STAMP(9);
     dec_accept = s_dec_accept;
     const unsigned vblock = s_vblock;
+    if (summed) claimSlices(s_dec_proceed && !s_dec_out.relin);
     main_wg = vblock == 0;
     if (vblock > 0) {
       constexpr int LP = THREADS / 4, CPP = LP / kSchurLandmarks;
@@ -410,7 +495,12 @@
     c_relin = a.ctrl->relin;
     lam = a.ctrl->lambda;
   }
+  if (!decides && summed) claimSlices(true);
   if (decides) eps_c = dec_eps;
+  if (summed) {
+    loadBatch(0);
+    if (tid < K) rhs_c = __hip_atomic_load(glb(a.comb_hand) + n_entries + tid, __ATOMIC_RELAXED, __HIP_MEMORY_SCOPE_AGENT);
+  }
   SC_STAMP(0);
   if (kStamps && a.dbg_stamps && tid == 0) a.dbg_stamps[7] = sc_t_entry;
   asm volatile("" : "+v"(fixed_c), "+v"(tomarg_c), "+v"(c_active), "+v"(c_relin));
@@ -431,6 +521,7 @@
   const int in_row = (tid >> 3) & 7, in_col = tid & 7;
   double *const A_thr = A + in_row * ld + in_col;
   auto storeBatch = [&](int base) {
+    awaitBatch(base);
     int blk = __builtin_amdgcn_readfirstlane((base + tid) >> 6);
     int bi, bj;
     combBlockDecode(blk, bi, bj);
@@ -469,6 +560,7 @@
   }
   SC_STAMP(11);
   if (tid < K) {
+    if (summed) awaitSlot(rhs_c, n_entries + tid);
     double v = rhs_c;
     if (prior_kind == 1)
       v += a.fixed_reg * eps_c;
@@ -484,6 +576,7 @@
   if (tid == 0) A[K * ld + K] = 0;
   ldsBarrier();
   SC_STAMP(1);
+  if (summed && s_comb_fault) return;
   if (main_wg) requestPairInputs();
 
   choleskyAugmented<THREADS>(A, pv, Linv, F, tid, a.dbg_stamps);
diff --git a/dsopp_amd/csrc/pba_solve_kernels.hpp b/dsopp_amd/csrc/pba_solve_kernels.hpp
--- a/dsopp_amd/csrc/pba_solve_kernels.hpp
+++ b/dsopp_amd/csrc/pba_solve_kernels.hpp
@@ -18,6 +18,7 @@
 constexpr int kSchurLandmarks = 64;
 constexpr int kSchurThreads = 512;
 constexpr int kPairBlk = 144;
+constexpr int kPairSlot = 208;
 
 __host__ __device__ inline int schurRowStride(int Kp) {
   return ((Kp + 15) / 32) * 32 + 16;
@@ -92,8 +93,9 @@
   double *scalars_out;
   int scalars_out_groups = 0;
   double *comb;
-  int comb_copies = 1;
-  int comb_copy_first = 0, comb_copy_stride = 0;
+  double *comb_parts = nullptr;
+  double *comb_pairs = nullptr;
+  int comb_part_stride = 0;
   double comb_lambda;
   LmParams prm;
   long long *dbg;
@@ -375,8 +377,8 @@
     hd_flags = d.flags;
   }
   asm volatile("" ::"s"(a.frames), "s"(a.Hpp), "s"(a.bpp), "s"(a.Hsc), "s"(a.bsc), "s"(a.for_marginalized), "s"(a.ublk_parity), "s"(a.ctrl_out),
-               "s"(a.st), "s"(a.scalars), "s"(a.n_sweep_blocks), "s"(a.scalars_out), "s"(a.scalars_out_groups), "s"(a.comb), "s"(a.comb_lambda), "s"(a.comb_copies),
-               "s"(a.comb_copy_first), "s"(a.comb_copy_stride));
+               "s"(a.st), "s"(a.scalars), "s"(a.n_sweep_blocks), "s"(a.scalars_out), "s"(a.scalars_out_groups), "s"(a.comb), "s"(a.comb_lambda), "s"(a.comb_parts),
+               "s"(a.comb_pairs), "s"(a.comb_part_stride));
   asm volatile("" : "+s"(hd.r), "+s"(hd.offset), "+s"(hd.n), "+s"(hd.cap), "+s"(hd_conn), "+s"(hd_ublk), "+s"(hd_flags), "+s"(c_active), "+s"(c_lsv),
                "+s"(comb_lam));
   if (!ctrl_p) {
@@ -392,9 +394,6 @@
   }
   if (!c_active || c_lsv) return;
   const int F = a.F, K = kBlk * F;
-  double *const comb_w = (a.comb && a.comb_copies > 1 && (blockIdx.x % a.comb_copies) != 0)
-                             ? a.comb + a.comb_copy_first + static_cast<size_t>(blockIdx.x % a.comb_copies - 1) * a.comb_copy_stride
-                             : a.comb;
   if (a.scalars_out && static_cast<int>(blockIdx.x) == a.n_schur_blocks + F * F) {
     double *lds = reinterpret_cast<double *>(smem_raw);
     double v[4] = {0, 0, 0, 0};
@@ -437,7 +436,15 @@
       if (lane < 48) wsum[wave * 48 + lane] = sw;
     }
     ldsBarrier();
-    if (threadIdx.x >= 64 || !valid) return;
+    if (threadIdx.x >= 64) return;
+    if (!valid) {
+      if (a.comb_pairs) {
+        double *slot = a.comb_pairs + static_cast<size_t>(p) * kPairSlot;
+        slot[lane] = slot[64 + lane] = slot[128 + lane] = 0;
+        if (lane < 16) slot[192 + lane] = 0;
+      }
+      return;
+    }
     double s = 0;
     if (lane < 44) {
 #pragma unroll
@@ -451,16 +458,28 @@
     __builtin_amdgcn_s_waitcnt(0);
     __builtin_amdgcn_wave_barrier();
     const int i = lane >> 3, j = lane & 7;
+    if (a.comb_pairs) {
+      double *slot = a.comb_pairs + static_cast<size_t>(p) * kPairSlot;
+      const double dl = i == j ? 1.0 + comb_lam : 1.0;
+      slot[lane] = dl * drv[lane];
+      slot[64 + lane] = dl * lds[symIdx(i, j)];
+      slot[128 + lane] = r > t ? -drv[64 + 8 * j + i] : -drv[64 + lane];
+      if (lane < 8) {
+        slot[192 + lane] = drv[128 + lane];
+        slot[200 + lane] = -lds[36 + lane];
+      }
+      return;
+    }
     if (a.comb) {
       const double dl = i == j ? 1.0 + comb_lam : 1.0;
-      atomicAdd(&comb_w[combBlockIndex(r, r) * 64 + lane], dl * drv[lane]);
-      atomicAdd(&comb_w[combBlockIndex(t, t) * 64 + lane], dl * lds[symIdx(i, j)]);
+      atomicAdd(&a.comb[combBlockIndex(r, r) * 64 + lane], dl * drv[lane]);
+      atomicAdd(&a.comb[combBlockIndex(t, t) * 64 + lane], dl * lds[symIdx(i, j)]);
       if (r > t)
-        atomicAdd(&comb_w[combBlockIndex(r, t) * 64 + lane], -drv[64 + 8 * j + i]);
+        atomicAdd(&a.comb[combBlockIndex(r, t) * 64 + lane], -drv[64 + 8 * j + i]);
       else
-        atomicAdd(&comb_w[combBlockIndex(t, r) * 64 + lane], -drv[64 + lane]);
+        atomicAdd(&a.comb[combBlockIndex(t, r) * 64 + lane], -drv[64 + lane]);
       if (lane < 8) {
-        double *rhs = comb_w + combBlockCount(F) * 64;
+        double *rhs = a.comb + combBlockCount(F) * 64;
         atomicAdd(&rhs[kBlk * r + lane], drv[128 + lane]);
         atomicAdd(&rhs[kBlk * t + lane], -lds[36 + lane]);
       }
@@ -515,6 +534,7 @@
   }
   for (int idx = threadIdx.x; idx < kSchurLandmarks * stride; idx += kSchurThreads) hrow[idx] = 0;
   double *Tm = wbd + kSchurLandmarks;
+  double *wscr = Tm;
   if (static_cast<int>(threadIdx.x) < F * 37) {
     const int t = threadIdx.x / 37, c = threadIdx.x - 37 * t;
     Tm[t * 40 + c] = tmv;
@@ -594,6 +614,7 @@
     const int nt = Kp >> 4;
     const int n_tiles = nt * (nt + 1) / 2;
     const int li = lane & 15, lk = lane >> 4;
+    double *const part = a.comb_parts ? a.comb_parts + static_cast<size_t>(blockIdx.x) * a.comb_part_stride : nullptr;
     for (int tile = wave; tile < n_tiles; tile += kSchurThreads / 64) {
       int ti = 0, rem = tile;
       while (rem >= nt - ti) {
@@ -618,14 +639,40 @@
       for (int reg = 0; reg < 4; ++reg) {
         const int row = 16 * ti + lk + 4 * reg, col = 16 * tj + li;
         const double v = acc[reg];
+        if (a.comb_parts) continue;
         if (a.comb) {
           const double sv = v * comb_sc;
-          if (row < K && col < K && col >= row && v != 0) atomicAdd(&comb_w[combIndex(col, row)], sv);
-          if (bd_in_pad && row < K && col == K && v != 0) atomicAdd(&comb_w[combBlockCount(F) * 64 + row], sv);
+          if (row < K && col < K && col >= row && v != 0) atomicAdd(&a.comb[combIndex(col, row)], sv);
+          if (bd_in_pad && row < K && col == K && v != 0) atomicAdd(&a.comb[combBlockCount(F) * 64 + row], sv);
           continue;
         }
         if (row < K && col < K && col >= row && v != 0) atomicAdd(&a.Hsc[row * K + col], v);
         if (bd_in_pad && row < K && col == K && v != 0) atomicAdd(&a.bsc[row], v);
+      }
+      if (a.comb_parts) {
+        double *scr = wscr + wave * 64;
+#pragma unroll
+        for (int q = 0; q < 4; ++q) {
+          if ((li >> 3) == (q >> 1)) {
+#pragma unroll
+            for (int h = 0; h < 2; ++h) {
+              const int reg = 2 * (q & 1) + h, rl = lk + 4 * reg;
+              scr[((li & 7) << 3) + (rl & 7)] = (ti == tj && li < rl) ? 0.0 : acc[reg] * comb_sc;
+            }
+          }
+          asm volatile("s_waitcnt lgkmcnt(0)" ::: "memory");
+          __builtin_amdgcn_wave_barrier();
+          const int bi = 2 * tj + (q >> 1), bj = 2 * ti + (q & 1);
+          const double sv = scr[lane];
+          if (bi < F && bj <= bi) part[combBlockIndex(bi, bj) * 64 + lane] = sv;
+          asm volatile("s_waitcnt lgkmcnt(0)" ::: "memory");
+          __builtin_amdgcn_wave_barrier();
+        }
+        if (bd_in_pad && 16 * tj + li == K) {
+#pragma unroll
+          for (int reg = 0; reg < 4; ++reg)
+            if (16 * ti + lk + 4 * reg < K) part[combBlockCount(F) * 64 + 16 * ti + lk + 4 * reg] = acc[reg] * comb_sc;
+        }
       }
     }
     RS_STAMP(4);
@@ -633,9 +680,11 @@
       double s = 0;
 #pragma unroll 1
       for (int ll = 0; ll < kSchurLandmarks; ++ll) s += wbd[ll] * hrow[ll * stride + c];
-      if (s != 0) {
+      if (a.comb_parts) {
+        part[combBlockCount(F) * 64 + c] = s * comb_sc;
+      } else if (s != 0) {
         if (a.comb)
-          atomicAdd(&comb_w[combBlockCount(F) * 64 + c], s * comb_sc);
+          atomicAdd(&a.comb[combBlockCount(F) * 64 + c], s * comb_sc);
         else
           atomicAdd(&a.bsc[c], s);
       }
```

Result: slower. 23720 GN iterations/s (-10.5%).
